# Chengyuann/AutoStyle-TTS

Hardware: AMD Instinct MI355X
Metric: synthesized audio sec/wall-sec (RTF^-1) + style-kNN QPS, IEMOCAP test batch (higher is better)
Workload: dtype f16; 1 GPU; BASELINE configs[1]: batch=8 utterances/GPU, kNN Q=8 x N=1000 x D=6144 k=3, synthesis Tt=32 Tp=150 Ts=250 (fixed-length decode, EOS ignored) -> 430 mel frames -> 110080 samples @ 22050 Hz; CosyVoice-300M shapes, random-init weights; parallelism=dp1 (model + bank replicated, utterances sharded, all-gather of style ids only)

## Files before the change

### autostyle-tts_amd/astts/_lib_session.py

```python
from __future__ import annotations

import functools
import os

from . import _lib

HEADER_PATH = os.path.normpath(os.path.join(os.path.dirname(os.path.abspath(__file__)), "..", "..", "include", "session",
                                            "astts_lm_session.h"))


@functools.lru_cache(maxsize=None)
def signatures() -> dict:
    if not os.path.exists(HEADER_PATH):
        raise _lib.AsttsLibraryMissing(f"{HEADER_PATH} not found: the ctypes signatures of the session calls are derived from this header")
    with open(HEADER_PATH) as f:
        return _lib.parse_prototypes(f.read())


@functools.lru_cache(maxsize=None)
def load():
    lib = _lib.load()
    for name, (res, args) in signatures().items():
        fn = getattr(lib, name)
        fn.restype = res
        fn.argtypes = args
    return lib
```

### autostyle-tts_amd/astts/synth/flow.py

```python
from __future__ import annotations

import ctypes
import math
from typing import List, NamedTuple, Optional

import torch

from .. import _lib, ops
from ..ops import PackedWeight
from .config import SynthConfig
from .encoder import SD, RelPosEncoder, _dev, fold_layernorm


class _Resnet1D:
    def __init__(self, sd: SD, p: str, device, groups: int):
        self.groups = groups
        self.c1 = PackedWeight.from_conv1d(sd[p + ".block1.block.0.weight"], sd[p + ".block1.block.0.bias"], device)
        self.g1 = (_dev(sd[p + ".block1.block.1.weight"], device), _dev(sd[p + ".block1.block.1.bias"], device))
        self.mlp = PackedWeight(sd[p + ".mlp.1.weight"], sd[p + ".mlp.1.bias"], device)
        self.c2 = PackedWeight.from_conv1d(sd[p + ".block2.block.0.weight"], sd[p + ".block2.block.0.bias"], device)
        self.g2 = (_dev(sd[p + ".block2.block.1.weight"], device), _dev(sd[p + ".block2.block.1.bias"], device))
        self.res = PackedWeight.from_conv1d(sd[p + ".res_conv.weight"], sd[p + ".res_conv.bias"], device)
        self.fused = all(w.cin == w.cin_pad for w in (self.c1, self.c2, self.res)) and \
            ops.resnet_conv_supported(self.c1.cin, self.c1.n, groups, self.c1.taps) and \
            ops.resnet_conv_supported(self.c2.cin, self.c2.n, groups, self.c2.taps) and \
            ops.resnet_conv_supported(self.res.cin, self.res.n, groups, self.res.taps)
        self.c1_frag, self.c2_frag, self.res_frag = ((ops.conv_pack_frag(self.c1), ops.conv_pack_frag(self.c2), ops.conv_pack_frag(self.res))
                                                     if self.fused else (None, None, None))

    def forward(self, x: torch.Tensor, lens: torch.Tensor, temb_mish: torch.Tensor, tproj: Optional[torch.Tensor] = None) -> torch.Tensor:
        if tproj is None:
            tproj = ops.linear(temb_mish, self.mlp)
        if self.fused:
            x = x.contiguous()
            h1, s1 = ops.resnet_conv(x, self.c1, self.c1_frag, lens=lens, want_stats=True)
            h2, s2 = ops.resnet_conv(h1, self.c2, self.c2_frag, lens=lens, in_gn=(s1, *self.g1), in_add=tproj.contiguous(), want_stats=True)
            return ops.resnet_conv(x, self.res, self.res_frag, lens=lens, res_gn=(h2, s2, *self.g2))
        h = ops.conv1d(x, self.c1, pad=1)
        h = ops.groupnorm(h, *self.g1, self.groups, 1e-5, lens=lens, mish=True, add_bc=tproj, out_dtype=torch.float16)
        h = ops.conv1d(h, self.c2, pad=1)
        h = ops.groupnorm(h, *self.g2, self.groups, 1e-5, lens=lens, mish=True)
        return ops.conv1d(x, self.res, residual=h)


class _TfmBlock:
    def __init__(self, sd: SD, p: str, heads: int, device):
        self.heads = heads
        wqkv = torch.cat([sd[p + ".attn1.to_q.weight"], sd[p + ".attn1.to_k.weight"], sd[p + ".attn1.to_v.weight"]], 0).float().cpu()
        wqkv, bqkv = fold_layernorm(wqkv, torch.zeros(wqkv.shape[0]), sd[p + ".norm1.weight"].float().cpu(), sd[p + ".norm1.bias"].float().cpu())
        c = int(wqkv.shape[1])
        self.n1 = (torch.ones(c, dtype=torch.float32, device=device), torch.zeros(c, dtype=torch.float32, device=device))
        self.wqkv = PackedWeight(wqkv, bqkv, device)
        self.wqkv_frag = ops.tfm_pack_frag(self.wqkv) if c == 256 and wqkv.shape[0] % 32 == 0 else None
        self.wo = PackedWeight(sd[p + ".attn1.to_out.0.weight"], sd[p + ".attn1.to_out.0.bias"], device)
        w1, b1 = fold_layernorm(sd[p + ".ff.net.0.proj.weight"].float().cpu(), sd[p + ".ff.net.0.proj.bias"].float().cpu(),
                                sd[p + ".norm3.weight"].float().cpu(), sd[p + ".norm3.bias"].float().cpu())
        self.n3 = self.n1
        self.w1 = PackedWeight(w1, b1, device)
        self.w2 = PackedWeight(sd[p + ".ff.net.2.weight"], sd[p + ".ff.net.2.bias"], device)
        self.ffn_fused = ops.tfm_ffn_fused_supported(c, int(w1.shape[0]))
        self.w1_frag = ops.tfm_pack_frag(self.w1) if self.ffn_fused else None
        self.w2_frag = ops.tfm_pack_frag(self.w2) if self.ffn_fused else None
        self.wo_frag = ops.tfm_pack_frag(self.wo) if self.ffn_fused and self.wo.cin in (256, 512) else None

    def forward(self, x: torch.Tensor, lens: torch.Tensor) -> torch.Tensor:
        hd = self.heads * 64
        f16 = torch.float16
        if self.wqkv_frag is not None and ops.tfm_attn_fused_supported(x.shape[-1], self.heads, x.shape[1]):
            a = ops.tfm_attn_fused(x, self.wqkv, self.wqkv_frag, self.heads, lens=lens, eps=1e-5)
        else:
            n = ops.layernorm(x, *self.n1, 1e-5, out_dtype=f16)
            qkv = ops.linear(n, self.wqkv, out_dtype=f16)
            a = ops.attn_mha(qkv[..., :hd], qkv[..., hd:2 * hd], qkv[..., 2 * hd:], self.heads, lens=lens, out_dtype=f16)
        if self.wo_frag is not None:
            return ops.tfm_ffn_fused(x, self.w1, self.w1_frag, self.w2, self.w2_frag, eps=1e-5, attn=a.contiguous(), wo=self.wo, wo_frag=self.wo_frag)
        x = ops.linear(a, self.wo, residual=x)
        if self.ffn_fused:
            return ops.tfm_ffn_fused(x, self.w1, self.w1_frag, self.w2, self.w2_frag, eps=1e-5)
        n = ops.layernorm(x, *self.n3, 1e-5, out_dtype=f16)
        f = ops.linear(n, self.w1, act="gelu", out_dtype=f16)
        return ops.linear(f, self.w2, residual=x)


class _Block(NamedTuple):
    res: _Resnet1D
    tfms: List[_TfmBlock]
    resample: Optional[PackedWeight] = None
    last: bool = False


class FlowDecoder:

    def __init__(self, sd: SD, cfg: SynthConfig, device):
        self.cfg, self.device = cfg, device
        self.use_engine = True
        self.tok_emb = _dev(sd["input_embedding.weight"], device)
        self.spk_aff = PackedWeight(sd["spk_embed_affine_layer.weight"], sd["spk_embed_affine_layer.bias"], device)
        self.enc = RelPosEncoder(sd, "encoder", cfg.flow_heads, cfg.flow_layers, "swish", ("norm_mha", "norm_ff"), False,
                                 False, cfg.ln_eps, cfg.max_positions, device)
        self.enc_proj = PackedWeight(sd["encoder_proj.weight"], sd["encoder_proj.bias"], device)
        self.lr = []
        for j in range(4):
            self.lr.append((PackedWeight.from_conv1d(sd[f"length_regulator.model.{3 * j}.weight"],
                                                     sd[f"length_regulator.model.{3 * j}.bias"], device),
                            _dev(sd[f"length_regulator.model.{3 * j + 1}.weight"], device),
                            _dev(sd[f"length_regulator.model.{3 * j + 1}.bias"], device)))
        self.lr_out = PackedWeight.from_conv1d(sd["length_regulator.model.12.weight"], sd["length_regulator.model.12.bias"], device)
        e = "decoder.estimator"
        self.t1 = PackedWeight(sd[e + ".time_mlp.linear_1.weight"], sd[e + ".time_mlp.linear_1.bias"], device)
        self.t2 = PackedWeight(sd[e + ".time_mlp.linear_2.weight"], sd[e + ".time_mlp.linear_2.bias"], device)
        ch = cfg.est_channels
        g = cfg.est_groups
        self.down, self.mid, self.up = [], [], []
        for i in range(len(ch)):
            p = f"{e}.down_blocks.{i}"
            last = i == len(ch) - 1
            wname = p + ".2" + ("" if last else ".conv")
            self.down.append(_Block(_Resnet1D(sd, p + ".0", device, g),
                                    [_TfmBlock(sd, f"{p}.1.{j}", cfg.est_heads, device) for j in range(cfg.est_tfm_per_block)],
                                    PackedWeight.from_conv1d(sd[wname + ".weight"], sd[wname + ".bias"], device), last))
        for i in range(cfg.est_mid_blocks):
            p = f"{e}.mid_blocks.{i}"
            self.mid.append(_Block(_Resnet1D(sd, p + ".0", device, g),
                                   [_TfmBlock(sd, f"{p}.1.{j}", cfg.est_heads, device) for j in range(cfg.est_tfm_per_block)]))
        for i in range(len(ch)):
            p = f"{e}.up_blocks.{i}"
            last = i == len(ch) - 1
            if last:
                w = PackedWeight.from_conv1d(sd[p + ".2.weight"], sd[p + ".2.bias"], device)
            else:
                w = PackedWeight.from_conv_transpose1d(sd[p + ".2.conv.weight"], sd[p + ".2.conv.bias"], 2, device)
            self.up.append(_Block(_Resnet1D(sd, p + ".0", device, g),
                                  [_TfmBlock(sd, f"{p}.1.{j}", cfg.est_heads, device) for j in range(cfg.est_tfm_per_block)], w, last))
        self.fin_c = PackedWeight.from_conv1d(sd[e + ".final_block.block.0.weight"], sd[e + ".final_block.block.0.bias"], device)
        self.fin_g = (_dev(sd[e + ".final_block.block.1.weight"], device), _dev(sd[e + ".final_block.block.1.bias"], device))
        self.fin_p = PackedWeight.from_conv1d(sd[e + ".final_proj.weight"], sd[e + ".final_proj.bias"], device)

    def mu(self, tokens: torch.Tensor, token_lens: torch.Tensor, mel_total: int, mel_lens: Optional[torch.Tensor] = None) -> torch.Tensor:
        x = ops.embedding(self.tok_emb, tokens.clamp(min=0))
        x = ops.elementwise(ops.EL_MUL_ROWMASK, x, lens=token_lens)
        h = ops.linear(self.enc.forward(x, token_lens), self.enc_proj)
        h = ops.interp_linear(h, mel_total, in_lens=None if mel_lens is None else token_lens, out_lens=mel_lens)
        for w, ga, be in self.lr:
            h = ops.conv1d(h, w, pad=1)
            h = ops.groupnorm(h, ga, be, 1, 1e-5, lens=mel_lens, mish=True)
        h = ops.conv1d(h, self.lr_out)
        return h if mel_lens is None else ops.elementwise(ops.EL_MUL_ROWMASK, h, lens=mel_lens)

    def time_path(self, t: torch.Tensor) -> List[torch.Tensor]:
        temb = ops.time_embedding(t, self.cfg.est_in)
        temb = ops.linear(ops.linear(temb, self.t1, act="silu"), self.t2)
        temb_m = ops.elementwise(ops.EL_MISH, temb)
        return [ops.linear(temb_m, blk.res.mlp) for grp in (self.down, self.mid, self.up) for blk in grp]

    def estimator(self, x, mu, spk, cond, t, lens, full: bool = False, tprojs: Optional[List[torch.Tensor]] = None) -> torch.Tensor:
        cfg = self.cfg
        b, T, _ = x.shape
        if full:
            _mask = lambda h, L: h
        else:
            _mask = lambda h, L: ops.elementwise(ops.EL_MUL_ROWMASK, h, lens=L)
        if tprojs is None:
            tprojs = self.time_path(t)
        tp = iter(tprojs)
        temb_m = None
        h = torch.cat([x, mu, spk[:, None, :].expand(b, T, -1), cond], dim=-1)
        hiddens, lens_stack = [], [lens]
        for res, tfms, wds, last in self.down:
            L = lens_stack[-1]
            h = _mask(h, L)
            h = res.forward(h, L, temb_m, next(tp))
            for tb in tfms:
                h = tb.forward(h, L)
            hiddens.append(h)
            hm = _mask(h, L)
            if last:
                h = ops.conv1d(hm, wds, pad=1)
                lens_stack.append(L)
            else:
                h = ops.conv1d(hm, wds, stride=2, pad=1)
                lens_stack.append(torch.div(L + 1, 2, rounding_mode="floor").to(torch.int32))
        L = lens_stack[-1]
        h = _mask(h, L)
        for blk in self.mid:
            h = blk.res.forward(h, L, temb_m, next(tp))
            for tb in blk.tfms:
                h = tb.forward(h, L)
            h = _mask(h, L)
        lens_stack.pop()
        for res, tfms, wus, last in self.up:
            L = lens_stack.pop()
            skip = hiddens.pop()
            h = torch.cat([h[:, :skip.shape[1]], skip], dim=-1)
            h = _mask(h, L)
            h = res.forward(h, L, temb_m, next(tp))
            for tb in tfms:
                h = tb.forward(h, L)
            hm = _mask(h, L)
            if last:
                h = ops.conv1d(hm, wus, pad=1)
            else:
                h = ops.conv_transpose1d(hm, wus, padding=1)
        h = _mask(h[:, :T].contiguous(), lens)
        h = ops.conv1d(h, self.fin_c, pad=1)
        h = ops.groupnorm(h, *self.fin_g, cfg.est_groups, 1e-5, lens=lens, mish=True)
        out = ops.conv1d(h, self.fin_p)
        return _mask(out, lens)

    def _engine(self):
        if getattr(self, "_eng", None) is None:
            cfg = self.cfg
            keep = []

            def W(pw):
                return ops.Weight(pw.data.data_ptr(), None if pw.bias is None else pw.bias.data_ptr(), pw.n, pw.cin, pw.cin_pad, pw.taps)

            def R(r):
                fp = [None if f is None else f.data_ptr() for f in (r.c1_frag, r.c2_frag, r.res_frag)]
                return ops.FlowResnet(W(r.c1), W(r.mlp), W(r.c2), W(r.res), r.g1[0].data_ptr(), r.g1[1].data_ptr(),
                                      r.g2[0].data_ptr(), r.g2[1].data_ptr(), *fp)

            def TF(tfms):
                arr = (ops.FlowTfm * len(tfms))()
                for i, t in enumerate(tfms):
                    arr[i] = ops.FlowTfm(t.n1[0].data_ptr(), t.n1[1].data_ptr(), t.n3[0].data_ptr(), t.n3[1].data_ptr(),
                                         W(t.wqkv), W(t.wo), W(t.w1), W(t.w2), None if t.wqkv_frag is None else t.wqkv_frag.data_ptr(),
                                         None if t.w1_frag is None else t.w1_frag.data_ptr(), None if t.w2_frag is None else t.w2_frag.data_ptr(),
                                         None if t.wo_frag is None else t.wo_frag.data_ptr())
                keep.append(arr)
                return arr

            def blocks(items, kinds):
                arr = (ops.FlowBlock * max(len(items), 1))()
                for i, (blk, kind) in enumerate(zip(items, kinds)):
                    rs = W(blk.resample) if kind != ops.FLOW_RESAMPLE_NONE else ops.Weight()
                    arr[i] = ops.FlowBlock(R(blk.res), TF(blk.tfms), len(blk.tfms), rs, kind)
                keep.append(arr)
                return arr

            down = blocks(self.down, [ops.FLOW_RESAMPLE_CONV if blk.last else ops.FLOW_RESAMPLE_DOWN for blk in self.down])
            mid = blocks(self.mid, [ops.FLOW_RESAMPLE_NONE] * len(self.mid))
            up = blocks(self.up, [ops.FLOW_RESAMPLE_CONV if blk.last else ops.FLOW_RESAMPLE_UP for blk in self.up])
            c = ops.FlowConfig(cfg.mel, cfg.est_channels[0], cfg.est_heads, cfg.est_groups, cfg.est_in, cfg.est_time_dim,
                               len(self.down), len(self.mid), len(self.up), W(self.t1), W(self.t2), W(self.fin_c), W(self.fin_p),
                               self.fin_g[0].data_ptr(), self.fin_g[1].data_ptr())
            h = ctypes.c_void_p()
            _lib.check(_lib.load().astts_flow_create(ctypes.byref(c), down, mid, up, ctypes.byref(h)))
            self._eng, self._eng_keep = h, keep
        return self._eng

    def _schedule(self):
        n = self.cfg.cfm_steps
        ts = 1.0 - torch.cos(torch.linspace(0, 1, n + 1) * 0.5 * math.pi)
        return [float(ts[s]) for s in range(n)], [float(ts[s + 1] - ts[s]) for s in range(n)]

    def solve(self, x: torch.Tensor, mu: torch.Tensor, spk_e: torch.Tensor, cond: torch.Tensor,
              lens: Optional[torch.Tensor] = None) -> torch.Tensor:
        lib = _lib.load()
        eng = self._engine()
        b, t, _ = x.shape
        assert x.is_contiguous() and mu.is_contiguous() and cond.is_contiguous() and spk_e.is_contiguous()
        assert x.dtype == mu.dtype == cond.dtype == spk_e.dtype == torch.float32
        tv, dv = self._schedule()
        n = len(tv)
        need = int(lib.astts_flow_workspace_bytes(eng, b, t))
        ws = torch.empty(need, dtype=torch.uint8, device=x.device)
        _lib.check(lib.astts_flow_solve(eng, x.data_ptr(), mu.data_ptr(), spk_e.data_ptr(), cond.data_ptr(),
                                        None if lens is None else lens.data_ptr(), b, t, n, (ctypes.c_float * n)(*tv),
                                        (ctypes.c_float * n)(*dv), self.cfg.cfg_rate, ws.data_ptr(), need,
                                        _lib.stream_ptr()))
        return x

    def solve_ops(self, x, mu, spk_e, cond, lens: Optional[torch.Tensor] = None) -> torch.Tensor:
        b, t, _ = x.shape
        full = lens is None
        if full:
            lens = torch.full((b,), t, dtype=torch.int32, device=x.device)
        lens2 = torch.cat([lens, lens])
        mu2 = torch.cat([mu, torch.zeros_like(mu)], 0)
        spk2 = torch.cat([spk_e, torch.zeros_like(spk_e)], 0)
        cond2 = torch.cat([cond, torch.zeros_like(cond)], 0)
        tv, dv = self._schedule()
        b2 = 2 * b
        t_all = torch.tensor(tv, dtype=torch.float32, device=x.device).repeat_interleave(b2)
        tp_all = self.time_path(t_all)
        for s in range(len(tv)):
            t2 = t_all[s * b2:(s + 1) * b2]
            d = self.estimator(torch.cat([x, x], 0), mu2, spk2, cond2, t2, lens2, full=full,
                               tprojs=[tp[s * b2:(s + 1) * b2] for tp in tp_all])
            x = ops.elementwise(ops.EL_CFG_EULER, x, z=d, s=dv[s], s2=self.cfg.cfg_rate)
        return x

    def decode(self, tokens, token_lens, prompt_mel, spk, z, mel_total: int) -> torch.Tensor:
        cfg = self.cfg
        b = tokens.shape[0]
        mu = self.mu(tokens, token_lens, mel_total)
        spk_e = ops.linear(torch.nn.functional.normalize(spk, dim=1), self.spk_aff)
        tmp = prompt_mel.shape[1]
        cond = torch.zeros((b, mel_total, cfg.mel), dtype=torch.float32, device=self.device)
        cond[:, :tmp] = prompt_mel
        x = (self.solve if self.use_engine else self.solve_ops)(z.clone(), mu, spk_e, cond)
        return x[:, tmp:].contiguous()

    def decode_ragged(self, tokens: List[torch.Tensor], prompt_mels: List[torch.Tensor], spk: torch.Tensor,
                      zs: List[torch.Tensor]) -> List[torch.Tensor]:
        cfg, dev = self.cfg, self.device
        b = len(tokens)
        tl = [int(t.numel()) for t in tokens]
        tmp = [int(m.shape[0]) for m in prompt_mels]
        mt = [int(z.shape[0]) for z in zs]
        tmax, mmax = max(tl), max(mt)
        tok = torch.zeros((b, tmax), dtype=torch.int32, device=dev)
        cond = torch.zeros((b, mmax, cfg.mel), dtype=torch.float32, device=dev)
        x = torch.zeros((b, mmax, cfg.mel), dtype=torch.float32, device=dev)
        for i in range(b):
            tok[i, :tl[i]] = tokens[i].to(dev).view(-1)
            cond[i, :tmp[i]] = prompt_mels[i].to(dev)
            x[i, :mt[i]] = zs[i].to(dev)
        tok_lens = torch.tensor(tl, dtype=torch.int32, device=dev)
        mel_lens = torch.tensor(mt, dtype=torch.int32, device=dev)
        mu = self.mu(tok, tok_lens, mmax, mel_lens)
        spk_e = ops.linear(torch.nn.functional.normalize(spk.to(dev), dim=1), self.spk_aff)
        x = (self.solve if self.use_engine else self.solve_ops)(x, mu, spk_e, cond, mel_lens)
        return [x[i, tmp[i]:mt[i]].contiguous() for i in range(b)]
```

### autostyle-tts_amd/astts/synth/pipeline.py

```python
from __future__ import annotations

import os
import threading
import time
from collections import deque
from concurrent.futures import Future, ThreadPoolExecutor
from typing import List, NamedTuple, Optional, Tuple

import torch

from .. import _lib, ops
from .decode import Prefill, record_streams
from .lm import AcousticLM

Slot = Optional[Tuple[int, int]]


def plan_streams(class_sizes: List[int], depth: int) -> Tuple[Slot, List[Slot], Slot]:
    n = len(class_sizes)
    if n >= depth + 2:
        return (0, 0), [(c, 0) for c in range(1, depth + 1)], (depth + 1, 0)
    front = (0, 1) if class_sizes[0] > 1 else None
    lm_classes = list(range(1, n)) if n > 1 else [0]
    lm = []
    for i in range(depth):
        c = lm_classes[i % len(lm_classes)]
        j = i // len(lm_classes) + (0 if n > 1 else 2)
        lm.append((c, j) if j < class_sizes[c] else None)
    return (0, 0), lm, front


class LmArgs(NamedTuple):
    text: torch.Tensor
    text_lens: torch.Tensor
    lm_spk: torch.Tensor
    lm_prompt_tokens: torch.Tensor
    n_tokens: int
    uniforms: torch.Tensor

    @property
    def rows(self) -> int:
        return int(self.text.shape[0])

    @classmethod
    def concat(cls, parts: List["LmArgs"]) -> "LmArgs":
        a = parts
        return cls(torch.cat([x.text for x in a], 0), torch.cat([x.text_lens for x in a], 0), torch.cat([x.lm_spk for x in a], 0),
                   torch.cat([x.lm_prompt_tokens for x in a], 0), a[0].n_tokens, torch.cat([x.uniforms for x in a], 1))


def _lib_check_spin(us: int, stream) -> None:
    _lib.check(_lib.load().astts_stream_spin(int(us), int(stream.cuda_stream)))


class _JoinChain:

    ROWS_MAX = 16

    def __init__(self, lm, device, stream, index: int, quantum: int, ahead: int, max_window: int):
        self.lm, self.device, self.stream, self.index = lm, device, stream, index
        self.quantum, self.ahead, self.max_window = quantum, ahead, max_window
        self.session = None
        self._cv = threading.Condition()
        self._waiting = deque()
        self._occupied = 0
        self._half = 0
        self._stop = False
        self._dead = None
        self._thread = None
        self.gate = threading.Event()
        self.gate.set()
        self.joins = 0

    def occupied(self) -> int:
        with self._cv:
            return self._occupied

    def reserve(self, window: int) -> bool:
        with self._cv:
            if self._dead is not None:
                raise RuntimeError(f"decode chain {self.index} stopped: {self._dead!r}") from self._dead
            if self._occupied >= 2 or window > self.max_window:
                return False
            if window > self._half:
                if self._occupied:
                    return False
                self._half = min((window + 127) // 128 * 128, self.max_window)
            self._occupied += 1
            return True

    def submit(self, state: Prefill, lm_args: LmArgs) -> Future:
        cur = torch.cuda.current_stream(self.device)
        record_streams(lm_args, self.stream)
        record_streams(state.tensors(), self.stream)
        ready = torch.cuda.Event()
        ready.record(cur)
        fut = Future()
        with self._cv:
            if self._dead is not None:
                self._occupied -= 1
                raise RuntimeError(f"decode chain {self.index} stopped: {self._dead!r}") from self._dead
            self._waiting.append((state, lm_args.uniforms, ready, fut))
            if self._thread is None:
                self._thread = threading.Thread(target=self._run, name=f"astts-join-chain-{self.index}", daemon=True)
                self._thread.start()
            self._cv.notify()
        return fut

    def close(self) -> None:
        with self._cv:
            self._stop = True
            self._cv.notify()
        self.gate.set()
        if self._thread is not None:
            self._thread.join()
            self._thread = None
        if self.session is not None:
            self.session.close()
            self.session = None

    def _admit_waiting(self, futs) -> None:
        while True:
            with self._cv:
                if not self._waiting:
                    return
                state, u, ready, fut = self._waiting[0]
                half = self._half
            idle = self.session is None or not self.session.active()
            if idle and (self.session is None or self.session.max_window < half):
                if self.session is not None:
                    self.session.close()
                    self.session = None
                self.session = self.lm.session(self.ROWS_MAX, 2 * half, self.stream)
            if not self.session.can_admit(state.b, state.s0, state.n_steps):
                if not idle:
                    return
                with self._cv:
                    self._waiting.popleft()
                    self._occupied -= 1
                fut.set_exception(RuntimeError(f"decode chain {self.index}: a batch of {state.b} rows with a window of "
                                               f"{state.s0 + state.n_steps - 1} keys does not fit a session of {self.ROWS_MAX} rows "
                                               f"and {self.session.max_window} keys"))
                continue
            self.joins += 0 if idle else 1
            self.stream.wait_event(ready)
            futs[id(self.session.admit(state, u, ignore_eos=True))] = fut
            with self._cv:
                self._waiting.popleft()

    def _run(self):
        ahead = deque()
        futs = {}
        try:
            with torch.cuda.device(self.device), torch.cuda.stream(self.stream):
                while True:
                    self.gate.wait()
                    with self._cv:
                        while not self._stop and not self._waiting and not (self.session is not None and self.session.active()):
                            self._cv.wait()
                        if self._stop:
                            return
                    self._admit_waiting(futs)
                    if not self.session.active():
                        continue
                    done = self.session.step(min(self.quantum, min(self.session.steps_left())))
                    mark = torch.cuda.Event()
                    mark.record(self.stream)
                    for job in done:
                        with self._cv:
                            self._occupied -= 1
                        futs.pop(id(job)).set_result(([job.toks], mark))
                    ahead.append(mark)
                    if len(ahead) > self.ahead:
                        ahead.popleft().synchronize()
        except BaseException as e:
            with self._cv:
                self._dead = e
                pending = [w[3] for w in self._waiting]
                self._waiting.clear()
                self._occupied = 0
            for f in list(futs.values()) + pending:
                if not f.done():
                    f.set_exception(e)


class PipelinedSynth:

    JOIN_QUANTUM = 16
    JOIN_AHEAD = 2

    def __init__(self, engine, lm_depth: int = 2, lm_priority: int = -1, render_priority: int = 0, streams=None,
                 cobatch: int = 1, render_depth: int = 1, pipe_classes=None, front_prefill: Optional[bool] = None,
                 stagger_ms: Optional[float] = None, wide_lm: bool = False, join: bool = False):
        self.eng = engine
        self.depth = max(1, int(lm_depth))
        self.render_depth = rd = max(1, int(render_depth))
        dev = engine.device
        with torch.cuda.device(dev):
            self.front_stream = None
            extra_render = []
            if streams is not None:
                self.s_lm, self.s_render = list(streams[:self.depth]), streams[self.depth]
                extra_render = list(streams[self.depth + 1:self.depth + rd])
            elif lm_priority != render_priority:
                self.s_lm = [torch.cuda.Stream(device=dev, priority=lm_priority) for _ in range(self.depth)]
                self.s_render = torch.cuda.Stream(device=dev, priority=render_priority)
            elif rd > 1:
                st = ops.concurrent_streams(self.depth + 1 + rd, priority=lm_priority, device=dev)
                self.s_render, extra_render, self.front_stream, self.s_lm = st[0], st[1:rd], st[rd], st[rd + 1:]
            else:
                classes = pipe_classes if pipe_classes is not None else ops.stream_pipe_classes(priority=lm_priority, device=dev)
                render, lm, front = plan_streams([len(c) for c in classes], self.depth)
                self.s_render = classes[render[0]][render[1]]
                self.s_lm = [torch.cuda.Stream(device=dev, priority=lm_priority) if s is None else classes[s[0]][s[1]] for s in lm]
                self.front_stream = None if front is None else classes[front[0]][front[1]]
            if self.front_stream is None:
                self.front_stream = torch.cuda.Stream(device=dev)
            while len(extra_render) < rd - 1:
                extra_render.append(torch.cuda.Stream(device=dev, priority=render_priority))
            self.s_renders = [self.s_render] + list(extra_render)
            self._r = 0
        self._pool = ThreadPoolExecutor(max_workers=self.depth)
        self._fifo = deque()
        self._pending = []
        self.cobatch = max(1, int(cobatch))
        self.wide_lm = bool(wide_lm)
        self.lm_rows_max = AcousticLM.WIDE_ROWS if self.wide_lm else 32
        self.front_prefill = (os.environ.get("ASTTS_PIPE_FRONT_PREFILL", "1") != "0") if front_prefill is None else bool(front_prefill)
        self.stagger_ms = float(os.environ.get("ASTTS_PIPE_STAGGER_MS", "0")) if stagger_ms is None else float(stagger_ms)
        self._staggered = set()
        self._i = 0
        self.join = bool(join) and self.cobatch == 1 and not self.wide_lm
        lm_ = engine.lm
        self._chains = [_JoinChain(lm_, dev, self.s_lm[c], c, self.JOIN_QUANTUM, self.JOIN_AHEAD, lm_.body.center)
                        for c in range(self.depth)] if self.join else []

    def close(self) -> None:
        for ch in self._chains:
            ch.close()
        self._chains = []
        self._pool.shutdown(wait=True)

    @classmethod
    def autotune(cls, engine, sample_args, depths=(3, 2), trials: int = 3, steps: int = 4, verbose: bool = False,
                 front=None, dist=None, wide_lm: bool = False):
        best, best_dt = None, float("inf")
        per_cfg = []
        with torch.cuda.device(engine.device):
            classes = ops.stream_pipe_classes(device=engine.device, verbose=verbose)
        tried = []
        for cfg_ in depths:
            cfg_ = cfg_ if isinstance(cfg_, tuple) else (cfg_, 1)
            for join in (False, True):
                if join and (cfg_[1] != 1 or wide_lm):
                    continue
                tried.append(tuple(cfg_) + ("join",) if join else cfg_)
        for cfg_ in tried:
            join = cfg_[-1] == "join"
            depth, cob, rdep = (tuple(cfg_[:-1] if join else cfg_) + (1,))[:3]
            for _ in range(trials):
                lm_prio = int(os.environ.get("ASTTS_PIPE_LM_PRIORITY", "0"))
                pipe = cls(engine, lm_depth=depth, lm_priority=lm_prio, render_priority=0, cobatch=cob, render_depth=rdep,
                           pipe_classes=classes if rdep == 1 and lm_prio == 0 else None, wide_lm=wide_lm, join=join)
                with torch.cuda.stream(pipe.front_stream):
                    for _ in range((depth + 1) * cob):
                        if front is not None:
                            front()
                        pipe.submit(*sample_args)
                    pipe.drain()
                    torch.cuda.synchronize(engine.device)
                    t0 = time.perf_counter()
                    for _ in range(steps):
                        if front is not None:
                            front()
                        pipe.submit(*sample_args)
                    pipe.drain()
                    torch.cuda.synchronize(engine.device)
                dt = (time.perf_counter() - t0) / steps
                if verbose:
                    print(f"PipelinedSynth.autotune: depth {depth} cobatch {cob} render streams {rdep} join {join}: {dt * 1e3:.1f} ms/batch", flush=True)
                if dt < best_dt:
                    best, best_dt = pipe, dt
                if not per_cfg or per_cfg[-1][2] != cfg_:
                    per_cfg.append([pipe, dt, cfg_])
                elif dt < per_cfg[-1][1]:
                    if per_cfg[-1][0] is not best:
                        per_cfg[-1][0].close()
                    per_cfg[-1][0], per_cfg[-1][1] = pipe, dt
                else:
                    pipe.close()
        if dist is not None and len(per_cfg) > 1:
            t = torch.tensor([c[1] for c in per_cfg], dtype=torch.float64, device=engine.device)
            dist.all_reduce(t, op=dist.ReduceOp.MAX)
            k = int(torch.argmin(t).item())
            best, best_dt = per_cfg[k][0], per_cfg[k][1]
            best.tuned_agreed_over_ranks = True
        for c in per_cfg:
            if c[0] is not best:
                c[0].close()
        best.tuned_ms_per_batch = best_dt * 1e3
        best.tuned_table_ms = {str(c[2]): round(c[1] * 1e3, 2) for c in per_cfg}
        return best

    def _launch_group(self):
        group, self._pending = self._pending, []
        chain = self._i % self.depth
        stream = self.s_lm[chain]
        self._i += 1
        cur = torch.cuda.current_stream(self.eng.device)
        if self.stagger_ms > 0 and chain > 0 and chain not in self._staggered:
            self._staggered.add(chain)
            us = int(self.stagger_ms * 1000.0 * chain)
            while us > 0:
                _lib_check_spin(min(us, 100000), stream)
                us -= 100000
        lm_args = group[0]["lm"] if len(group) == 1 else LmArgs.concat([g["lm"] for g in group])
        record_streams(lm_args, stream)
        sizes = [g["lm"].rows for g in group]
        state = None
        if self.front_prefill and sum(sizes) <= self.lm_rows_max:
            state = self.eng.tts_prefill(*lm_args[:5])
            record_streams(state.tensors(), stream)
        stream.wait_stream(cur)

        def lm_stage():
            with torch.cuda.device(self.eng.device), torch.cuda.stream(stream):
                toks = self.eng.tts_tokens(*lm_args, wide=self.wide_lm) if state is None else self.eng.tts_decode(state, lm_args.uniforms)
                parts = list(torch.split(toks, sizes, 0)) if len(sizes) > 1 else [toks]
                ev = torch.cuda.Event()
                ev.record(stream)
            return parts, ev

        fut = self._pool.submit(lm_stage)
        for k, g in enumerate(group):
            g["fut"], g["k"] = fut, k

    def _render(self, item):
        parts, ev = item["fut"].result()
        toks = parts[item["k"]]
        cur = torch.cuda.current_stream(self.eng.device)
        sr = self.s_renders[self._r % self.render_depth]
        self._r += 1
        with torch.cuda.stream(sr):
            sr.wait_event(ev)
            toks.record_stream(sr)
            record_streams(item["render"], sr)
            mel, wav = self.eng.tts_render(toks, *item["render"])
        record_streams((toks, mel, wav), cur)
        return toks, mel, wav

    def submit(self, text, text_lens, lm_spk, lm_prompt_tokens, n_tokens, uniforms, flow_prompt_tokens, flow_prompt_mel,
               flow_spk, z, phase0, noise):
        cur = torch.cuda.current_stream(self.eng.device)
        for sr in self.s_renders:
            sr.wait_stream(cur)
        item = {"lm": LmArgs(text, text_lens, lm_spk, lm_prompt_tokens, n_tokens, uniforms),
                "render": (flow_prompt_tokens, flow_prompt_mel, flow_spk, z, phase0, noise), "fut": None, "k": 0}
        if self.join and self._join_submit(item):
            return self._render(self._fifo.popleft()) if len(self._fifo) > 2 * self.depth else None
        if self._pending and not self._compatible(self._pending[0]["lm"], item["lm"]):
            self._launch_group()
        self._pending.append(item)
        self._fifo.append(item)
        if len(self._pending) >= self.cobatch:
            self._launch_group()
        if len(self._fifo) > self.depth * self.cobatch and self._fifo[0]["fut"] is not None:
            return self._render(self._fifo.popleft())
        return None

    def _join_submit(self, item) -> bool:
        lm, lm_args = self.eng.lm, item["lm"]
        if lm_args.rows > _JoinChain.ROWS_MAX // 2:
            return False
        pre = lm.prefix(lm_args.text, lm_args.text_lens, lm_args.lm_spk, lm_args.lm_prompt_tokens)
        window = int(pre.shape[0]) + int(lm_args.n_tokens) - 1
        if window > lm.body.center:
            return False
        state = lm.prefill(pre, lm_args.n_tokens)
        order = lambda: sorted(self._chains, key=lambda ch: (ch.occupied() != 1, ch.index))
        chain = next((ch for ch in order() if ch.reserve(window)), None)
        for older in list(self._fifo):
            if chain is not None:
                break
            if older["fut"] is not None:
                try:
                    older["fut"].result()
                except Exception:
                    pass
                chain = next((ch for ch in order() if ch.reserve(window)), None)
        if chain is None:
            raise RuntimeError("PipelinedSynth: no decode chain can take the batch although none holds one")
        self._fifo.append(item)
        item["fut"] = chain.submit(state, lm_args)
        return True

    def _compatible(self, a: LmArgs, b: LmArgs) -> bool:
        return (a.n_tokens == b.n_tokens and a.text.shape[1] == b.text.shape[1]
                and a.lm_prompt_tokens.shape[1] == b.lm_prompt_tokens.shape[1] and a.uniforms.shape[0] == b.uniforms.shape[0]
                and a.rows + b.rows <= self.lm_rows_max)

    def drain(self):
        if self._pending:
            self._launch_group()
        self._staggered = set()
        self._i = 0
        out = []
        while self._fifo:
            out.append(self._render(self._fifo.popleft()))
        cur = torch.cuda.current_stream(self.eng.device)
        for st in self.s_lm:
            cur.wait_stream(st)
        for sr in self.s_renders:
            cur.wait_stream(sr)
        return out
```

### autostyle-tts_amd/csrc/flow_engine.hip

```cpp
#include "common.h"

#include <vector>

struct astts_flow {
    astts_flow_config_t cfg;
    struct Block {
        astts_flow_resnet_t res;
        std::vector<astts_flow_tfm_t> tfm;
        astts_weight_t resample;
        int kind;
    };
    std::vector<Block> down, mid, up;
};

namespace astts {

__global__ __launch_bounds__(256) void flow_pack_input(const float* __restrict__ x, const float* __restrict__ mu,
                                                      const float* __restrict__ spk, const float* __restrict__ cond,
                                                      const int* __restrict__ lens2, float* __restrict__ out, int b, int t,
                                                      int mel) {
    const int c4 = 4 * mel;
    const int64_t total = (int64_t)2 * b * t * c4;
    for (int64_t i = (int64_t)blockIdx.x * blockDim.x + threadIdx.x; i < total; i += (int64_t)gridDim.x * blockDim.x) {
        const int c = (int)(i % c4);
        const int64_t row = i / c4;
        const int bb = (int)(row / t), tt = (int)(row % t);
        const int src_b = bb < b ? bb : bb - b;
        const int part = c / mel, cc = c % mel;
        float v = 0.0f;
        if (tt < lens2[bb]) {
            const int64_t o = ((int64_t)src_b * t + tt) * mel + cc;
            if (part == 0) v = x[o];
            else if (bb < b) v = part == 1 ? mu[o] : (part == 2 ? spk[(int64_t)src_b * mel + cc] : cond[o]);
        }
        out[i] = v;
    }
}

__global__ __launch_bounds__(256) void flow_concat_skip(const float* __restrict__ a, int64_t a_bs, const float* __restrict__ skip,
                                                       const int* __restrict__ lens, float* __restrict__ out, int b2, int t, int c) {
    const int c4 = c / 4;
    const int64_t total = (int64_t)b2 * t * 2 * c4;
    for (int64_t i = (int64_t)blockIdx.x * blockDim.x + threadIdx.x; i < total; i += (int64_t)gridDim.x * blockDim.x) {
        const int cc = (int)(i % (2 * c4));
        const int64_t row = i / (2 * c4);
        const int bb = (int)(row / t), tt = (int)(row % t);
        float4 v = make_float4(0.f, 0.f, 0.f, 0.f);
        if (tt < lens[bb]) {
            if (cc < c4) v = reinterpret_cast<const float4*>(a + (int64_t)bb * a_bs + (int64_t)tt * c)[cc];
            else v = reinterpret_cast<const float4*>(skip + row * c)[cc - c4];
        }
        reinterpret_cast<float4*>(out)[i] = v;
    }
}

__global__ void flow_fill_lens(const int* __restrict__ lens, int* __restrict__ lens_full, int* __restrict__ lens_half, int b, int t) {
    const int i = blockIdx.x * blockDim.x + threadIdx.x;
    if (i < 2 * b) {
        const int l = lens ? lens[i < b ? i : i - b] : t;
        lens_full[i] = l;
        lens_half[i] = (l + 1) / 2;
    }
}

__global__ void flow_fill_time(float* __restrict__ tv, float value, int n) {
    const int i = blockIdx.x * blockDim.x + threadIdx.x;
    if (i < n) tv[i] = value;
}

static inline int grid_for(int64_t total) {
    int64_t g = (total + 255) / 256;
    return (int)(g > 8192 ? 8192 : g);
}

}

using namespace astts;

#define RUN(expr)                          \
    do {                                   \
        const int rc_ = (expr);            \
        if (rc_ != ASTTS_OK) return rc_;   \
    } while (0)

namespace {

constexpr int FLOW_MAX_STEPS = 32;

struct Buffers {
    float *xin, *r1, *r2, *r3, *pool[6], *temb0, *temb1, *temb2, *tproj, *tv, *d, *up;
    _Float16 *r1h, *n16, *qkv16, *a16, *f16;
    int *lens_full, *lens_half;
    void* gn_ws;
    size_t gn_ws_bytes;
    float *rstat1, *rstat2;
};

size_t carve(const astts_flow* h, int b, int t, char* base, Buffers* B) {
    const astts_flow_config_t& c = h->cfg;
    const size_t b2 = 2 * (size_t)b, rows = b2 * t, C = c.channels, hd = (size_t)c.heads * 64;
    size_t o = 0;
    auto take = [&](size_t bytes) {
        void* p = base ? base + o : nullptr;
        o = align_up(o + bytes, 256);
        return p;
    };
    const size_t in_ch = 4 * (size_t)c.mel > 2 * C ? 4 * (size_t)c.mel : 2 * C;
    Buffers tmp;
    Buffers& X = B ? *B : tmp;
    X.xin = (float*)take(sizeof(float) * rows * in_ch);
    X.r1 = (float*)take(sizeof(float) * rows * C);
    X.r2 = (float*)take(sizeof(float) * rows * C);
    X.r3 = (float*)take(sizeof(float) * rows * C);
    for (int i = 0; i < 6; ++i) X.pool[i] = (float*)take(sizeof(float) * rows * C);
    X.up = (float*)take(sizeof(float) * b2 * ((size_t)t + 4) * 2 * C);
    X.r1h = (_Float16*)take(sizeof(_Float16) * rows * C);
    X.n16 = (_Float16*)take(sizeof(_Float16) * rows * C);
    X.qkv16 = (_Float16*)take(sizeof(_Float16) * rows * 3 * hd);
    X.a16 = (_Float16*)take(sizeof(_Float16) * rows * hd);
    X.f16 = (_Float16*)take(sizeof(_Float16) * rows * 4 * C);
    const size_t n_res = h->down.size() + h->mid.size() + h->up.size();
    X.temb0 = (float*)take(sizeof(float) * FLOW_MAX_STEPS * b2 * c.time_in);
    X.temb1 = (float*)take(sizeof(float) * FLOW_MAX_STEPS * b2 * c.time_dim);
    X.temb2 = (float*)take(sizeof(float) * FLOW_MAX_STEPS * b2 * c.time_dim);
    X.tproj = (float*)take(sizeof(float) * n_res * FLOW_MAX_STEPS * b2 * C);
    X.tv = (float*)take(sizeof(float) * FLOW_MAX_STEPS * b2);
    X.d = (float*)take(sizeof(float) * rows * c.mel);
    X.lens_full = (int*)take(sizeof(int) * b2);
    X.lens_half = (int*)take(sizeof(int) * b2);
    X.gn_ws_bytes = astts_op_groupnorm_workspace_bytes((int)b2, t, c.groups);
    X.gn_ws = take(X.gn_ws_bytes > 16 ? X.gn_ws_bytes : 16);
    X.rstat1 = (float*)take(sizeof(float) * astts_op_resnet_conv_stats_floats((int32_t)b2, t));
    X.rstat2 = (float*)take(sizeof(float) * astts_op_resnet_conv_stats_floats((int32_t)b2, t));
    return o;
}

struct Ctx {
    const astts_flow* h;
    Buffers B;
    int b2, T;
    bool full;
    astts_stream_t st;

    int gemm(const void* x, int x16, const astts_weight_t& w, const float* residual, void* out, int out16, int64_t m,
             int t_in, int t_out, int stride, int pad, int act) const {
        return astts_op_gemm(x, x16, w.w, w.bias, residual, nullptr, out, out16, m, w.n, w.cin, w.cin_pad, w.taps, w.cin, w.n,
                             residual ? w.n : 0, t_in, t_out, stride, 1, pad, act, 1.0f, 0.1f, nullptr, st);
    }
    int linear(const void* x, int x16, const astts_weight_t& w, const float* residual, void* out, int out16, int64_t m, int act) const {
        return gemm(x, x16, w, residual, out, out16, m, (int)m, (int)m, 1, 0, act);
    }
    int mask(float* x, const int* lens, int t, int c) const {
        if (full) return ASTTS_OK;
        return astts_op_elementwise(ASTTS_EL_MUL_ROWMASK, x, nullptr, nullptr, lens, x, (int64_t)b2 * t * c, t, c, 0.0f, 0.0f, st);
    }

    int resnet(const astts_flow_resnet_t& r, const float* tproj, const float* x, const int* lens, int t, float* out,
               const void* next_w = nullptr, uint32_t next_bytes = 0) const {
        const int C = h->cfg.channels, G = h->cfg.groups;
        const int64_t rows = (int64_t)b2 * t;
        if (r.c1_frag && r.c2_frag && r.res_frag && astts_op_resnet_conv_supported(r.c1.cin, r.c1.n, G, r.c1.taps) &&
            astts_op_resnet_conv_supported(r.c2.cin, r.c2.n, G, r.c2.taps) && astts_op_resnet_conv_supported(r.res.cin, r.res.n, G, r.res.taps)) {
            auto wbytes = [](const astts_weight_t& w) { return (uint32_t)((size_t)w.n * w.taps * w.cin_pad * 2); };
            RUN(astts_op_resnet_conv(x, r.c1_frag, r.c1.bias, B.r1, nullptr, nullptr, nullptr, nullptr, nullptr, nullptr, nullptr, nullptr,
                                     B.rstat1, lens, b2, t, r.c1.cin, r.c1.taps, 1e-5f, r.c2_frag, wbytes(r.c2), st));
            RUN(astts_op_resnet_conv(B.r1, r.c2_frag, r.c2.bias, B.r2, B.rstat1, r.g1_w, r.g1_b, tproj, nullptr, nullptr, nullptr, nullptr,
                                     B.rstat2, lens, b2, t, r.c2.cin, r.c2.taps, 1e-5f, r.res_frag, wbytes(r.res), st));
            return astts_op_resnet_conv(x, r.res_frag, r.res.bias, out, nullptr, nullptr, nullptr, nullptr, B.r2, B.rstat2, r.g2_w, r.g2_b,
                                        nullptr, lens, b2, t, r.res.cin, r.res.taps, 1e-5f, next_w, next_bytes, st);
        }
        RUN(gemm(x, 0, r.c1, nullptr, B.r1, 0, rows, t, t, 1, 1, ASTTS_ACT_NONE));
        RUN(astts_op_groupnorm(B.r1, lens, r.g1_w, r.g1_b, tproj, B.r1h, 1, b2, t, C, G, 1e-5f, 1, B.gn_ws, B.gn_ws_bytes, st));
        RUN(gemm(B.r1h, 1, r.c2, nullptr, B.r2, 0, rows, t, t, 1, 1, ASTTS_ACT_NONE));
        RUN(astts_op_groupnorm(B.r2, lens, r.g2_w, r.g2_b, nullptr, B.r3, 0, b2, t, C, G, 1e-5f, 1, B.gn_ws, B.gn_ws_bytes, st));
        return gemm(x, 0, r.res, B.r3, out, 0, rows, t, t, 1, 0, ASTTS_ACT_NONE);
    }

    int tfm(const astts_flow_tfm_t& w, float* p, float* q, const int* lens, int t, const void* next_w = nullptr, uint32_t next_bytes = 0) const {
        const int C = h->cfg.channels, heads = h->cfg.heads, hd = heads * 64;
        const int64_t rows = (int64_t)b2 * t;
        static const int64_t unfused_min = exp_env_int("ASTTS_FLOW_UNFUSED_ATTN_MIN_ROWS", 0);
        const bool fused_attn = w.qkv_frag && astts_op_tfm_attn_fused_supported(C, heads, t) && !(unfused_min > 0 && rows >= unfused_min);
        if (fused_attn) {
            const void* pf[3] = {w.wo_frag, w.w1_frag, w.w2_frag};
            const uint32_t pfb[3] = {(uint32_t)((size_t)C * hd * 2), (uint32_t)((size_t)w.w1.n * C * 2), (uint32_t)((size_t)C * w.w1.n * 2)};
            RUN(astts_op_tfm_attn_fused(p, w.qkv_frag, w.qkv.bias, lens, B.a16, b2, heads, t, C, 1e-5f, 0.125f, pf, pfb,
                                        (w.wo_frag && w.w1_frag && w.w2_frag) ? 3 : 0, st));
        } else {
            RUN(astts_op_layernorm(p, w.n1_w, w.n1_b, B.n16, 1, rows, C, C, C, 1e-5f, 0.0f, st));
            RUN(linear(B.n16, 1, w.qkv, nullptr, B.qkv16, 1, rows, ASTTS_ACT_NONE));
            RUN(astts_op_attn_mha(B.qkv16, B.qkv16 + hd, B.qkv16 + 2 * hd, 1, lens, B.a16, 1, b2, heads, t, 3 * hd, 3 * hd, hd,
                                  0.125f, st));
        }
        const bool ffn = w.w1_frag && w.w2_frag && astts_op_tfm_ffn_fused_supported(C, w.w1.n);
        if (ffn && w.wo_frag && (hd == 256 || hd == 512))
            return astts_op_tfm_ffn_fused(p, w.w1_frag, w.w1.bias, w.w2_frag, w.w2.bias, p, rows, C, w.w1.n, 1e-5f, B.a16, w.wo_frag,
                                          w.wo.bias, hd, next_w, next_bytes, st);
        RUN(linear(B.a16, 1, w.wo, p, q, 0, rows, ASTTS_ACT_NONE));
        if (ffn)
            return astts_op_tfm_ffn_fused(q, w.w1_frag, w.w1.bias, w.w2_frag, w.w2.bias, p, rows, C, w.w1.n, 1e-5f, nullptr, nullptr, nullptr, 0, nullptr, 0,
                                          st);
        RUN(astts_op_layernorm(q, w.n3_w, w.n3_b, B.n16, 1, rows, C, C, C, 1e-5f, 0.0f, st));
        RUN(linear(B.n16, 1, w.w1, nullptr, B.f16, 1, rows, ASTTS_ACT_GELU));
        return linear(B.f16, 1, w.w2, q, p, 0, rows, ASTTS_ACT_NONE);
    }
};

}

extern "C" {

int astts_flow_create(const astts_flow_config_t* cfg, const astts_flow_block_t* down, const astts_flow_block_t* mid,
                      const astts_flow_block_t* up, astts_flow_t** out) {
    ASTTS_REQUIRE(cfg && down && mid && up && out, ASTTS_ERR_INVALID, "astts_flow_create: null argument");
    ASTTS_REQUIRE(cfg->mel >= 1 && cfg->channels >= 64 && cfg->channels % 64 == 0 && cfg->heads >= 1 && cfg->groups >= 1 &&
                      cfg->channels % cfg->groups == 0, ASTTS_ERR_INVALID, "astts_flow_create: bad sizes");
    ASTTS_REQUIRE(cfg->n_down >= 1 && cfg->n_down <= 4 && cfg->n_up == cfg->n_down && cfg->n_mid >= 0, ASTTS_ERR_INVALID,
                  "astts_flow_create: n_down=%d n_mid=%d n_up=%d", cfg->n_down, cfg->n_mid, cfg->n_up);
    int n_half = 0;
    for (int i = 0; i < cfg->n_down; ++i) n_half += down[i].resample_kind == ASTTS_FLOW_RESAMPLE_DOWN;
    ASTTS_REQUIRE(n_half <= 1, ASTTS_ERR_UNSUPPORTED, "astts_flow_create: more than one stride-2 level is not implemented");
    ASTTS_REQUIRE(down[cfg->n_down - 1].resample_kind == ASTTS_FLOW_RESAMPLE_CONV && up[cfg->n_up - 1].resample_kind == ASTTS_FLOW_RESAMPLE_CONV,
                  ASTTS_ERR_UNSUPPORTED, "astts_flow_create: the last down / up block must end in the k=3 convolution");
    astts_flow* h = new astts_flow();
    h->cfg = *cfg;
    auto copy = [](const astts_flow_block_t* src, int n, std::vector<astts_flow::Block>& dst) {
        for (int i = 0; i < n; ++i) {
            astts_flow::Block blk;
            blk.res = src[i].res;
            blk.tfm.assign(src[i].tfm, src[i].tfm + src[i].n_tfm);
            blk.resample = src[i].resample;
            blk.kind = src[i].resample_kind;
            dst.push_back(blk);
        }
    };
    copy(down, cfg->n_down, h->down);
    copy(mid, cfg->n_mid, h->mid);
    copy(up, cfg->n_up, h->up);
    *out = h;
    return ASTTS_OK;
}

int astts_flow_destroy(astts_flow_t* h) {
    delete h;
    return ASTTS_OK;
}

size_t astts_flow_workspace_bytes(const astts_flow_t* h, int32_t b, int32_t t) {
    if (!h || b < 1 || t < 1) return 0;
    return carve(h, b, t, nullptr, nullptr);
}

int astts_flow_solve(astts_flow_t* h, float* x, const float* mu, const float* spk, const float* cond, const int32_t* lens,
                     int32_t b, int32_t t, int32_t n_steps, const float* t_host, const float* dt_host, float cfg_rate,
                     void* workspace, size_t workspace_bytes, astts_stream_t stream) {
    ASTTS_REQUIRE(h && x && mu && spk && cond && t_host && dt_host && workspace, ASTTS_ERR_INVALID, "astts_flow_solve: null argument");
    ASTTS_REQUIRE(b >= 1 && t >= 2 && n_steps >= 1, ASTTS_ERR_INVALID, "astts_flow_solve: b=%d t=%d n_steps=%d", b, t, n_steps);
    ASTTS_REQUIRE(workspace_bytes >= astts_flow_workspace_bytes(h, b, t) && ((uintptr_t)workspace & 255) == 0,
                  ASTTS_ERR_WORKSPACE, "astts_flow_solve: workspace too small or misaligned");
    const astts_flow_config_t& c = h->cfg;
    hipStream_t st = (hipStream_t)stream;
    Ctx k;
    k.h = h;
    k.b2 = 2 * b;
    k.T = t;
    k.full = lens == nullptr;
    k.st = stream;
    carve(h, b, t, (char*)workspace, &k.B);
    const Buffers& B = k.B;
    const int b2 = k.b2, C = c.channels, mel = c.mel;
    const int t_half = (t - 1) / 2 + 1;

    hipLaunchKernelGGL(flow_fill_lens, dim3((b2 + 63) / 64), dim3(64), 0, st, lens, B.lens_full, B.lens_half, b, t);
    ASTTS_CHECK_LAUNCH();

    for (int s = 0; s < n_steps; ++s) {
      const int s0 = s - s % FLOW_MAX_STEPS, sl = s - s0;
      const int64_t trows = (int64_t)(n_steps - s0 < FLOW_MAX_STEPS ? n_steps - s0 : FLOW_MAX_STEPS) * b2;
      if (sl == 0) {
        for (int j = 0; j < (int)(trows / b2); ++j) {
            hipLaunchKernelGGL(flow_fill_time, dim3((b2 + 63) / 64), dim3(64), 0, st, B.tv + (size_t)j * b2, t_host[s0 + j], b2);
            ASTTS_CHECK_LAUNCH();
        }
        RUN(astts_op_time_embedding(B.tv, B.temb0, (int)trows, c.time_in, 1000.0f, st));
        RUN(k.linear(B.temb0, 0, c.t1, nullptr, B.temb1, 0, trows, ASTTS_ACT_SILU));
        RUN(k.linear(B.temb1, 0, c.t2, nullptr, B.temb2, 0, trows, ASTTS_ACT_NONE));
        RUN(astts_op_elementwise(ASTTS_EL_MISH, B.temb2, nullptr, nullptr, nullptr, B.temb2, trows * c.time_dim, 1, c.time_dim, 0.0f, 0.0f, st));
        size_t rj = 0;
        for (const std::vector<astts_flow::Block>* grp : {&h->down, &h->mid, &h->up})
            for (const astts_flow::Block& blk : *grp)
                RUN(k.linear(B.temb2, 0, blk.res.mlp, nullptr, B.tproj + (rj++) * (size_t)trows * C, 0, trows, ASTTS_ACT_NONE));
      }
      {
        size_t ri = 0;
        auto tproj_of = [&]() { return B.tproj + ((ri++) * (size_t)trows + (size_t)sl * b2) * C; };
        hipLaunchKernelGGL(flow_pack_input, dim3(grid_for((int64_t)b2 * t * 4 * mel)), dim3(256), 0, st, x, mu, spk, cond,
                           B.lens_full, B.xin, b, t, mel);
        ASTTS_CHECK_LAUNCH();

        float* pool[6];
        for (int i = 0; i < 6; ++i) pool[i] = B.pool[i];
        int n_free = 6;
        auto grab = [&]() { return pool[--n_free]; };
        float* cur = grab();
        float* other = grab();
        float* skips[4];
        int skip_t[4];
        const int* skip_lens[4];
        int n_skips = 0;
        const float* block_in = B.xin;
        int tt = t;
        const int* L = B.lens_full;

        const uint32_t qkv_bytes = 3u * (uint32_t)c.heads * 64u * (uint32_t)C * 2u;
        for (size_t i = 0; i < h->down.size(); ++i) {
            const astts_flow::Block& blk = h->down[i];
            RUN(k.resnet(blk.res, tproj_of(), block_in, L, tt, other, blk.tfm.empty() ? nullptr : blk.tfm[0].qkv_frag, qkv_bytes));
            { float* sw = cur; cur = other; other = sw; }
            for (size_t ti = 0; ti < blk.tfm.size(); ++ti) {
                const bool more = ti + 1 < blk.tfm.size();
                RUN(k.tfm(blk.tfm[ti], cur, other, L, tt, more ? blk.tfm[ti + 1].qkv_frag : nullptr,
                          more ? (uint32_t)(3u * (uint32_t)c.heads * 64u * (uint32_t)C * 2u) : 0u));
            }
            RUN(k.mask(cur, L, tt, C));
            skips[n_skips] = cur;
            skip_t[n_skips] = tt;
            skip_lens[n_skips] = L;
            ++n_skips;
            float* nxt = other;
            other = grab();
            if (blk.kind == ASTTS_FLOW_RESAMPLE_DOWN) {
                RUN(k.gemm(cur, 0, blk.resample, nullptr, nxt, 0, (int64_t)b2 * t_half, tt, t_half, 2, 1, ASTTS_ACT_NONE));
                tt = t_half;
                L = B.lens_half;
            } else {
                RUN(k.gemm(cur, 0, blk.resample, nullptr, nxt, 0, (int64_t)b2 * tt, tt, tt, 1, 1, ASTTS_ACT_NONE));
            }
            cur = nxt;
            RUN(k.mask(cur, L, tt, C));
            block_in = cur;
        }
        for (size_t mi = 0; mi < h->mid.size(); ++mi) {
            const astts_flow::Block& blk = h->mid[mi];
            RUN(k.resnet(blk.res, tproj_of(), cur, L, tt, other, blk.tfm.empty() ? nullptr : blk.tfm[0].qkv_frag, qkv_bytes));
            float* sw = cur; cur = other; other = sw;
            for (size_t ti = 0; ti < blk.tfm.size(); ++ti) {
                const bool more = ti + 1 < blk.tfm.size();
                const astts_flow_resnet_t* nr = (!more && mi + 1 < h->mid.size()) ? &h->mid[mi + 1].res : nullptr;
                const astts_weight_t* nc = nr ? &nr->c1 : nullptr;
                const void* nw = !nr ? nullptr
                                 : (nr->c1_frag && nr->c2_frag && nr->res_frag && astts_op_resnet_conv_supported(nc->cin, nc->n, c.groups, nc->taps) &&
                                    astts_op_resnet_conv_supported(nr->c2.cin, nr->c2.n, c.groups, nr->c2.taps) &&
                                    astts_op_resnet_conv_supported(nr->res.cin, nr->res.n, c.groups, nr->res.taps)) ? nr->c1_frag : nc->w;
                RUN(k.tfm(blk.tfm[ti], cur, other, L, tt, more ? blk.tfm[ti + 1].qkv_frag : nw,
                          more ? (uint32_t)(3u * (uint32_t)c.heads * 64u * (uint32_t)C * 2u)
                               : (nc ? (uint32_t)((size_t)nc->n * nc->taps * nc->cin_pad * 2) : 0u)));
            }
            RUN(k.mask(cur, L, tt, C));
        }
        const float* up_src = cur;
        int64_t up_bs = (int64_t)tt * C;
        for (size_t i = 0; i < h->up.size(); ++i) {
            const astts_flow::Block& blk = h->up[i];
            --n_skips;
            tt = skip_t[n_skips];
            L = skip_lens[n_skips];
            hipLaunchKernelGGL(flow_concat_skip, dim3(grid_for((int64_t)b2 * tt * 2 * (C / 4))), dim3(256), 0, st, up_src, up_bs,
                               skips[n_skips], L, B.xin, b2, tt, C);
            ASTTS_CHECK_LAUNCH();
            RUN(k.resnet(blk.res, tproj_of(), B.xin, L, tt, cur, blk.tfm.empty() ? nullptr : blk.tfm[0].qkv_frag, qkv_bytes));
            for (size_t ti = 0; ti < blk.tfm.size(); ++ti) {
                const bool more = ti + 1 < blk.tfm.size();
                RUN(k.tfm(blk.tfm[ti], cur, other, L, tt, more ? blk.tfm[ti + 1].qkv_frag : nullptr,
                          more ? (uint32_t)(3u * (uint32_t)c.heads * 64u * (uint32_t)C * 2u) : 0u));
            }
            RUN(k.mask(cur, L, tt, C));
            if (blk.kind == ASTTS_FLOW_RESAMPLE_UP) {
                RUN(k.gemm(cur, 0, blk.resample, nullptr, B.up, 0, (int64_t)b2 * (tt + 1), tt, tt + 1, 1, 1, ASTTS_ACT_NONE));
                up_src = B.up + C;
                up_bs = (int64_t)(tt + 1) * 2 * C;
            } else {
                RUN(k.gemm(cur, 0, blk.resample, nullptr, other, 0, (int64_t)b2 * tt, tt, tt, 1, 1, ASTTS_ACT_NONE));
                float* sw = cur; cur = other; other = sw;
                up_src = cur;
                up_bs = (int64_t)tt * C;
            }
        }
        float* fin = const_cast<float*>(up_src);
        RUN(k.mask(fin, B.lens_full, t, C));
        RUN(k.gemm(fin, 0, c.fin_c, nullptr, B.r1, 0, (int64_t)b2 * t, t, t, 1, 1, ASTTS_ACT_NONE));
        RUN(astts_op_groupnorm(B.r1, B.lens_full, c.fin_g_w, c.fin_g_b, nullptr, B.r3, 0, b2, t, C, c.groups, 1e-5f, 1, B.gn_ws,
                               B.gn_ws_bytes, st));
        RUN(k.gemm(B.r3, 0, c.fin_p, nullptr, B.d, 0, (int64_t)b2 * t, t, t, 1, 0, ASTTS_ACT_NONE));
        RUN(k.mask(B.d, B.lens_full, t, mel));
        RUN(astts_op_elementwise(ASTTS_EL_CFG_EULER, x, B.d, nullptr, nullptr, x, (int64_t)b * t * mel, t, mel, dt_host[s], cfg_rate, st));
      }
    }
    return ASTTS_OK;
}

}
```

Before: 521.8 audio-s/wall-s.

## Add continuous-batching flow session that joins render jobs across estimator passes

Adds a native flow-matching session holding up to four in-flight render jobs. Each estimator pass runs over all active jobs' rows together, and a new job can be admitted mid-solve. A background render thread feeds finished LM outputs into this session instead of running a separate full ODE solve per batch. The goal is larger, better-filled estimator GEMMs and less serialization between LM and render stages. The cost is extra threading, a per-pass join/assemble kernel and host-side scheduling overhead. It is only active in autotune candidates that pick render_join.

After: 537.4 audio-s/wall-s (median of 6 runs). 1.03x the previous value.

```diff
diff --git a/autostyle-tts_amd/astts/_lib_session.py b/autostyle-tts_amd/astts/_lib_session.py
--- a/autostyle-tts_amd/astts/_lib_session.py
+++ b/autostyle-tts_amd/astts/_lib_session.py
@@ -5,16 +5,20 @@
 
 from . import _lib
 
-HEADER_PATH = os.path.normpath(os.path.join(os.path.dirname(os.path.abspath(__file__)), "..", "..", "include", "session",
-                                            "astts_lm_session.h"))
+_DIR = os.path.normpath(os.path.join(os.path.dirname(os.path.abspath(__file__)), "..", "..", "include", "session"))
+HEADER_PATH = os.path.join(_DIR, "astts_lm_session.h")
+FLOW_HEADER_PATH = os.path.join(_DIR, "astts_flow_session.h")
 
 
 @functools.lru_cache(maxsize=None)
 def signatures() -> dict:
-    if not os.path.exists(HEADER_PATH):
-        raise _lib.AsttsLibraryMissing(f"{HEADER_PATH} not found: the ctypes signatures of the session calls are derived from this header")
-    with open(HEADER_PATH) as f:
-        return _lib.parse_prototypes(f.read())
+    sigs = {}
+    for path in (HEADER_PATH, FLOW_HEADER_PATH):
+        if not os.path.exists(path):
+            raise _lib.AsttsLibraryMissing(f"{path} not found: the ctypes signatures of the session calls are derived from this header")
+        with open(path) as f:
+            sigs.update(_lib.parse_prototypes(f.read()))
+    return sigs
 
 
 @functools.lru_cache(maxsize=None)
diff --git a/autostyle-tts_amd/astts/synth/flow.py b/autostyle-tts_amd/astts/synth/flow.py
--- a/autostyle-tts_amd/astts/synth/flow.py
+++ b/autostyle-tts_amd/astts/synth/flow.py
@@ -302,6 +302,18 @@
         x = (self.solve if self.use_engine else self.solve_ops)(z.clone(), mu, spk_e, cond)
         return x[:, tmp:].contiguous()
 
+    def session(self, t: int, slots: int = 4, rows_max: int = 32, stream=None) -> "FlowSession":
+        return FlowSession(self, t, slots, rows_max, stream)
+
+    def prepare(self, tokens, token_lens, prompt_mel, spk, z, mel_total: int):
+        b = tokens.shape[0]
+        mu = self.mu(tokens, token_lens, mel_total)
+        spk_e = ops.linear(torch.nn.functional.normalize(spk, dim=1), self.spk_aff)
+        tmp = prompt_mel.shape[1]
+        cond = torch.zeros((b, mel_total, self.cfg.mel), dtype=torch.float32, device=self.device)
+        cond[:, :tmp] = prompt_mel
+        return z.clone(), mu, spk_e, cond, tmp
+
     def decode_ragged(self, tokens: List[torch.Tensor], prompt_mels: List[torch.Tensor], spk: torch.Tensor,
                       zs: List[torch.Tensor]) -> List[torch.Tensor]:
         cfg, dev = self.cfg, self.device
@@ -323,3 +335,85 @@
         spk_e = ops.linear(torch.nn.functional.normalize(spk.to(dev), dim=1), self.spk_aff)
         x = (self.solve if self.use_engine else self.solve_ops)(x, mu, spk_e, cond, mel_lens)
         return [x[i, tmp[i]:mt[i]].contiguous() for i in range(b)]
+
+
+class FlowJob:
+
+    def __init__(self, x, mu, spk_e, cond, lens, n_steps: int):
+        self.x, self.mu, self.spk_e, self.cond, self.lens = x, mu, spk_e, cond, lens
+        self.n_steps, self.next, self.slot = int(n_steps), 0, -1
+
+
+class FlowSession:
+
+    def __init__(self, flow: FlowDecoder, t: int, slots: int = 4, rows_max: int = 32, stream=None):
+        from .. import _lib_session
+        self.flow, self.t, self.slots, self.rows_max = flow, int(t), int(slots), int(rows_max)
+        self.stream = stream if stream is not None else torch.cuda.current_stream(flow.device)
+        self._lib = _lib_session.load()
+        self._tv, self._dv = flow._schedule()
+        eng = flow._engine()
+        need = int(self._lib.astts_flow_session_bytes(eng, self.t, self.slots, self.rows_max, len(self._tv)))
+        if need == 0:
+            raise ValueError(f"FlowSession: t={t} slots={slots} rows_max={rows_max} steps={len(self._tv)}")
+        with torch.cuda.stream(self.stream):
+            self._ws = torch.empty(need, dtype=torch.uint8, device=flow.device)
+        h = ctypes.c_void_p()
+        _lib.check(self._lib.astts_flow_session_create(eng, self.t, self.slots, self.rows_max, len(self._tv), self._ws.data_ptr(), need,
+                                                       _lib.stream_ptr(self.stream), ctypes.byref(h)))
+        self._h = h
+        self._ctx: List[Optional[FlowJob]] = [None] * 4
+
+    def close(self) -> None:
+        if self._h is not None:
+            h, self._h = self._h, None
+            _lib.check(self._lib.astts_flow_session_destroy(h))
+
+    def active(self) -> int:
+        return sum(c is not None for c in self._ctx)
+
+    def steps_left(self) -> List[int]:
+        return [c.n_steps - c.next for c in self._ctx if c is not None]
+
+    def can_admit(self, b: int, t: int) -> bool:
+        return int(self._lib.astts_flow_session_can_admit(self._h, int(b), int(t), len(self._tv))) >= 0
+
+    def state(self) -> List[int]:
+        out = (ctypes.c_int32 * 8)()
+        _lib.check(self._lib.astts_flow_session_state(self._h, out))
+        return list(out)
+
+    def admit(self, x: torch.Tensor, mu: torch.Tensor, spk_e: torch.Tensor, cond: torch.Tensor,
+              lens: Optional[torch.Tensor] = None) -> FlowJob:
+        b, t, _ = x.shape
+        assert x.is_contiguous() and mu.is_contiguous() and cond.is_contiguous() and spk_e.is_contiguous()
+        assert x.dtype == mu.dtype == cond.dtype == spk_e.dtype == torch.float32
+        n = len(self._tv)
+        job = FlowJob(x, mu, spk_e, cond, lens, n)
+        slot = ctypes.c_int32(-1)
+        with torch.cuda.stream(self.stream):
+            _lib.check(self._lib.astts_flow_session_admit(self._h, x.data_ptr(), mu.data_ptr(), spk_e.data_ptr(), cond.data_ptr(),
+                                                          None if lens is None else lens.data_ptr(), b, t, n, (ctypes.c_float * n)(*self._tv),
+                                                          (ctypes.c_float * n)(*self._dv), self.flow.cfg.cfg_rate, ctypes.byref(slot)))
+        job.slot = int(slot.value)
+        self._ctx[job.slot] = job
+        return job
+
+    def step(self, k: int = 1) -> List[FlowJob]:
+        mask = ctypes.c_uint32(0)
+        k = int(k)
+        with torch.cuda.stream(self.stream):
+            _lib.check(self._lib.astts_flow_session_step(self._h, k, ctypes.byref(mask)))
+        done = []
+        for slot, c in enumerate(self._ctx):
+            if c is None:
+                continue
+            c.next = min(c.n_steps, c.next + k)
+            if mask.value >> slot & 1:
+                done.append(c)
+                self._ctx[slot] = None
+        return done
+
+    def run(self) -> None:
+        while self.active():
+            self.step(max(self.steps_left()))
diff --git a/autostyle-tts_amd/astts/synth/pipeline.py b/autostyle-tts_amd/astts/synth/pipeline.py
--- a/autostyle-tts_amd/astts/synth/pipeline.py
+++ b/autostyle-tts_amd/astts/synth/pipeline.py
@@ -184,14 +184,145 @@
                     f.set_exception(e)
 
 
+class _JoinRender:
+
+    SLOTS, ROWS_MAX, AHEAD = 4, 32, 2
+
+    def __init__(self, engine, stream):
+        self.eng, self.device, self.stream = engine, engine.device, stream
+        self.session = None
+        self._cv = threading.Condition()
+        self._waiting = []
+        self._stop = False
+        self._dead = None
+        self._thread = None
+        self.passes = self.carried = 0
+        self.gate = threading.Event()
+        self.gate.set()
+
+    def submit(self, item, ready) -> None:
+        item["rfut"], item["ready"] = Future(), ready
+        with self._cv:
+            if self._dead is not None:
+                raise RuntimeError(f"render worker stopped: {self._dead!r}") from self._dead
+            self._waiting.append(item)
+            if self._thread is None:
+                self._thread = threading.Thread(target=self._run, name="astts-join-render", daemon=True)
+                self._thread.start()
+        item["fut"].add_done_callback(self._wake)
+
+    def _wake(self, _fut=None) -> None:
+        with self._cv:
+            self._cv.notify()
+
+    def stats(self):
+        s = self.session.state() if self.session is not None else [0] * 8
+        return self.passes + s[2], self.carried + s[3]
+
+    def close(self) -> None:
+        with self._cv:
+            self._stop = True
+            self._cv.notify()
+        self.gate.set()
+        if self._thread is not None:
+            self._thread.join()
+            self._thread = None
+        self._drop_session()
+
+    def _drop_session(self) -> None:
+        if self.session is not None:
+            self.passes, self.carried = self.stats()
+            self.session.close()
+            self.session = None
+
+    def _take_ready(self):
+        busy = self.session is not None and self.session.active() > 0
+        with self._cv:
+            for i, item in enumerate(self._waiting):
+                fut = item["fut"]
+                if fut.done() and (not busy or fut.exception() is not None or fut.result()[1].query()):
+                    return self._waiting.pop(i)
+        return None
+
+    def _begin(self, item, jobs) -> None:
+        eng, sr = self.eng, self.stream
+        try:
+            parts, ev = item["fut"].result()
+        except Exception as e:
+            item["rfut"].set_exception(e)
+            return
+        toks = parts[item["k"]]
+        sr.wait_event(ev)
+        sr.wait_event(item["ready"])
+        toks.record_stream(sr)
+        record_streams(item["render"], sr)
+        ptok, pmel, spk, z, phase0, noise = item["render"]
+        b = int(toks.shape[0])
+        mel_total = int(pmel.shape[1]) + eng.cfg.mel_frames_for_tokens(toks.shape[1])
+        idle = self.session is None or not self.session.active()
+        if idle and b <= self.ROWS_MAX and (self.session is None or self.session.t != mel_total):
+            self._drop_session()
+            self.session = eng.flow.session(mel_total, self.SLOTS, self.ROWS_MAX, sr)
+        if not eng.flow.use_engine or self.session is None or not self.session.can_admit(b, mel_total):
+            mel, wav = eng.tts_render(toks, *item["render"])
+            item["rfut"].set_result((toks, mel, wav))
+            return
+        all_tok = torch.cat([ptok.to(torch.int32), toks], dim=1)
+        tok_lens = torch.full((b,), all_tok.shape[1], dtype=torch.int32, device=self.device)
+        x, mu, spk_e, cond, tmp = eng.flow.prepare(all_tok, tok_lens, pmel, spk, z, mel_total)
+        jobs[id(self.session.admit(x, mu, spk_e, cond))] = (item, toks, tmp)
+
+    def _run(self):
+        ahead = deque()
+        jobs = {}
+        item = None
+        try:
+            with torch.cuda.device(self.device), torch.cuda.stream(self.stream):
+                while True:
+                    self.gate.wait()
+                    with self._cv:
+                        while not self._stop and not (self.session is not None and self.session.active()) and \
+                                not any(w["fut"].done() for w in self._waiting):
+                            self._cv.wait()
+                        if self._stop:
+                            return
+                    while True:
+                        item = self._take_ready()
+                        if item is None:
+                            break
+                        self._begin(item, jobs)
+                        item = None
+                    if self.session is None or not self.session.active():
+                        continue
+                    for job in self.session.step(1):
+                        it, toks, tmp = jobs.pop(id(job))
+                        mel = job.x[:, tmp:].contiguous()
+                        wav = self.eng.hift.forward(mel, it["render"][4], it["render"][5])
+                        it["rfut"].set_result((toks, mel, wav))
+                    mark = torch.cuda.Event()
+                    mark.record(self.stream)
+                    ahead.append(mark)
+                    if len(ahead) > self.AHEAD:
+                        ahead.popleft().synchronize()
+        except BaseException as e:
+            with self._cv:
+                self._dead = e
+                held = [w for w in self._waiting] + [j[0] for j in jobs.values()] + ([item] if item is not None else [])
+                self._waiting.clear()
+            for it in held:
+                if not it["rfut"].done():
+                    it["rfut"].set_exception(e)
+
+
 class PipelinedSynth:
 
     JOIN_QUANTUM = 16
     JOIN_AHEAD = 2
+    AUTOTUNE_RENDER_JOIN = os.environ.get("ASTTS_PIPE_RENDER_JOIN", "1") != "0"
 
     def __init__(self, engine, lm_depth: int = 2, lm_priority: int = -1, render_priority: int = 0, streams=None,
                  cobatch: int = 1, render_depth: int = 1, pipe_classes=None, front_prefill: Optional[bool] = None,
-                 stagger_ms: Optional[float] = None, wide_lm: bool = False, join: bool = False):
+                 stagger_ms: Optional[float] = None, wide_lm: bool = False, join: bool = False, render_join: bool = False):
         self.eng = engine
         self.depth = max(1, int(lm_depth))
         self.render_depth = rd = max(1, int(render_depth))
@@ -234,11 +365,15 @@
         lm_ = engine.lm
         self._chains = [_JoinChain(lm_, dev, self.s_lm[c], c, self.JOIN_QUANTUM, self.JOIN_AHEAD, lm_.body.center)
                         for c in range(self.depth)] if self.join else []
+        self.render_join = bool(render_join) and rd == 1
+        self._renderer = _JoinRender(engine, self.s_render) if self.render_join else None
 
     def close(self) -> None:
         for ch in self._chains:
             ch.close()
         self._chains = []
+        if self._renderer is not None:
+            self._renderer.close()
         self._pool.shutdown(wait=True)
 
     @classmethod
@@ -255,13 +390,15 @@
                 if join and (cfg_[1] != 1 or wide_lm):
                     continue
                 tried.append(tuple(cfg_) + ("join",) if join else cfg_)
+                if join and cls.AUTOTUNE_RENDER_JOIN and len(cfg_) < 3:
+                    tried.append(tuple(cfg_) + ("join", "render_join"))
         for cfg_ in tried:
-            join = cfg_[-1] == "join"
-            depth, cob, rdep = (tuple(cfg_[:-1] if join else cfg_) + (1,))[:3]
+            join, rjoin = "join" in cfg_, "render_join" in cfg_
+            depth, cob, rdep = (tuple(c for c in cfg_ if not isinstance(c, str)) + (1,))[:3]
             for _ in range(trials):
                 lm_prio = int(os.environ.get("ASTTS_PIPE_LM_PRIORITY", "0"))
                 pipe = cls(engine, lm_depth=depth, lm_priority=lm_prio, render_priority=0, cobatch=cob, render_depth=rdep,
-                           pipe_classes=classes if rdep == 1 and lm_prio == 0 else None, wide_lm=wide_lm, join=join)
+                           pipe_classes=classes if rdep == 1 and lm_prio == 0 else None, wide_lm=wide_lm, join=join, render_join=rjoin)
                 with torch.cuda.stream(pipe.front_stream):
                     for _ in range((depth + 1) * cob):
                         if front is not None:
@@ -278,7 +415,7 @@
                     torch.cuda.synchronize(engine.device)
                 dt = (time.perf_counter() - t0) / steps
                 if verbose:
-                    print(f"PipelinedSynth.autotune: depth {depth} cobatch {cob} render streams {rdep} join {join}: {dt * 1e3:.1f} ms/batch", flush=True)
+                    print(f"PipelinedSynth.autotune: depth {depth} cobatch {cob} render streams {rdep} join {join} render join {rjoin}: {dt * 1e3:.1f} ms/batch", flush=True)
                 if dt < best_dt:
                     best, best_dt = pipe, dt
                 if not per_cfg or per_cfg[-1][2] != cfg_:
@@ -334,8 +471,17 @@
         fut = self._pool.submit(lm_stage)
         for k, g in enumerate(group):
             g["fut"], g["k"] = fut, k
+            self._to_renderer(g)
+
+    def _to_renderer(self, item) -> None:
+        if self._renderer is not None:
+            self._renderer.submit(item, item["ready"])
 
     def _render(self, item):
+        if self._renderer is not None:
+            out = item["rfut"].result()
+            record_streams(out, torch.cuda.current_stream(self.eng.device))
+            return out
         parts, ev = item["fut"].result()
         toks = parts[item["k"]]
         cur = torch.cuda.current_stream(self.eng.device)
@@ -352,11 +498,19 @@
     def submit(self, text, text_lens, lm_spk, lm_prompt_tokens, n_tokens, uniforms, flow_prompt_tokens, flow_prompt_mel,
                flow_spk, z, phase0, noise):
         cur = torch.cuda.current_stream(self.eng.device)
-        for sr in self.s_renders:
-            sr.wait_stream(cur)
         item = {"lm": LmArgs(text, text_lens, lm_spk, lm_prompt_tokens, n_tokens, uniforms),
                 "render": (flow_prompt_tokens, flow_prompt_mel, flow_spk, z, phase0, noise), "fut": None, "k": 0}
+        if self._renderer is None:
+            for sr in self.s_renders:
+                sr.wait_stream(cur)
+        else:
+            item["ready"] = torch.cuda.Event()
+            item["ready"].record(cur)
         if self.join and self._join_submit(item):
+            if self._renderer is not None:
+                rfut = self._fifo[0].get("rfut")
+                done = rfut is not None and (rfut.done() or len(self._fifo) > 2 * self.depth + _JoinRender.SLOTS)
+                return self._render(self._fifo.popleft()) if done else None
             return self._render(self._fifo.popleft()) if len(self._fifo) > 2 * self.depth else None
         if self._pending and not self._compatible(self._pending[0]["lm"], item["lm"]):
             self._launch_group()
@@ -392,6 +546,7 @@
             raise RuntimeError("PipelinedSynth: no decode chain can take the batch although none holds one")
         self._fifo.append(item)
         item["fut"] = chain.submit(state, lm_args)
+        self._to_renderer(item)
         return True
 
     def _compatible(self, a: LmArgs, b: LmArgs) -> bool:
diff --git a/autostyle-tts_amd/csrc/flow_engine.hip b/autostyle-tts_amd/csrc/flow_engine.hip
--- a/autostyle-tts_amd/csrc/flow_engine.hip
+++ b/autostyle-tts_amd/csrc/flow_engine.hip
@@ -1,4 +1,6 @@
 #include "common.h"
+#include "flow_session.h"
+#include "../../include/session/astts_flow_session.h"
 
 #include <vector>
 
@@ -135,20 +137,58 @@
     return o;
 }
 
+struct Seg {
+    float* x;
+    const float *mu, *spk, *cond;
+    int seq0, b;
+    float dt, cfg_rate;
+};
+
 struct Ctx {
     const astts_flow* h;
     Buffers B;
     int b2, T;
     bool full;
     astts_stream_t st;
-
+    const Seg* seg;
+    int n_seg;
+
+    int gemm1(const void* x, int x16, const astts_weight_t& w, const float* residual, void* out, int out16, int64_t m,
+              int t_in, int t_out, int stride, int pad, int act) const {
+        return astts_op_gemm(x, x16, w.w, w.bias, residual, nullptr, out, out16, m, w.n, w.cin, w.cin_pad, w.taps, w.cin, w.n,
+                             residual ? w.n : 0, t_in, t_out, stride, 1, pad, act, 1.0f, 0.1f, nullptr, st);
+    }
     int gemm(const void* x, int x16, const astts_weight_t& w, const float* residual, void* out, int out16, int64_t m,
              int t_in, int t_out, int stride, int pad, int act) const {
-        return astts_op_gemm(x, x16, w.w, w.bias, residual, nullptr, out, out16, m, w.n, w.cin, w.cin_pad, w.taps, w.cin, w.n,
-                             residual ? w.n : 0, t_in, t_out, stride, 1, pad, act, 1.0f, 0.1f, nullptr, st);
+        if (n_seg == 1) return gemm1(x, x16, w, residual, out, out16, m, t_in, t_out, stride, pad, act);
+        for (int i = 0; i < n_seg; ++i) {
+            const int64_t s0 = seg[i].seq0, nb = 2 * (int64_t)seg[i].b;
+            RUN(gemm1((const char*)x + s0 * t_in * w.cin * (x16 ? 2 : 4), x16, w, residual ? residual + s0 * t_out * w.n : nullptr,
+                      (char*)out + s0 * t_out * w.n * (out16 ? 2 : 4), out16, nb * t_out, t_in, t_out, stride, pad, act));
+        }
+        return ASTTS_OK;
     }
     int linear(const void* x, int x16, const astts_weight_t& w, const float* residual, void* out, int out16, int64_t m, int act) const {
-        return gemm(x, x16, w, residual, out, out16, m, (int)m, (int)m, 1, 0, act);
+        return gemm1(x, x16, w, residual, out, out16, m, (int)m, (int)m, 1, 0, act);
+    }
+    int linear_seq(const void* x, int x16, const astts_weight_t& w, const float* residual, void* out, int out16, int t, int act) const {
+        if (n_seg == 1) return linear(x, x16, w, residual, out, out16, (int64_t)b2 * t, act);
+        for (int i = 0; i < n_seg; ++i) {
+            const int64_t r0 = (int64_t)seg[i].seq0 * t, m = 2 * (int64_t)seg[i].b * t;
+            RUN(linear((const char*)x + r0 * w.cin * (x16 ? 2 : 4), x16, w, residual ? residual + r0 * w.n : nullptr,
+                       (char*)out + r0 * w.n * (out16 ? 2 : 4), out16, m, act));
+        }
+        return ASTTS_OK;
+    }
+    int gnorm(const float* x, const int* lens, const float* gw, const float* gb, const float* add_bc, void* y, int y16, int t) const {
+        const int C = h->cfg.channels, G = h->cfg.groups;
+        for (int i = 0; i < n_seg; ++i) {
+            const int64_t s0 = n_seg == 1 ? 0 : seg[i].seq0;
+            const int nb = n_seg == 1 ? b2 : 2 * seg[i].b;
+            RUN(astts_op_groupnorm(x + s0 * t * C, lens + s0, gw, gb, add_bc ? add_bc + s0 * C : nullptr, (char*)y + s0 * t * C * (y16 ? 2 : 4),
+                                   y16, nb, t, C, G, 1e-5f, 1, B.gn_ws, B.gn_ws_bytes, st));
+        }
+        return ASTTS_OK;
     }
     int mask(float* x, const int* lens, int t, int c) const {
         if (full) return ASTTS_OK;
@@ -157,7 +197,7 @@
 
     int resnet(const astts_flow_resnet_t& r, const float* tproj, const float* x, const int* lens, int t, float* out,
                const void* next_w = nullptr, uint32_t next_bytes = 0) const {
-        const int C = h->cfg.channels, G = h->cfg.groups;
+        const int G = h->cfg.groups;
         const int64_t rows = (int64_t)b2 * t;
         if (r.c1_frag && r.c2_frag && r.res_frag && astts_op_resnet_conv_supported(r.c1.cin, r.c1.n, G, r.c1.taps) &&
             astts_op_resnet_conv_supported(r.c2.cin, r.c2.n, G, r.c2.taps) && astts_op_resnet_conv_supported(r.res.cin, r.res.n, G, r.res.taps)) {
@@ -170,9 +210,9 @@
                                         nullptr, lens, b2, t, r.res.cin, r.res.taps, 1e-5f, next_w, next_bytes, st);
         }
         RUN(gemm(x, 0, r.c1, nullptr, B.r1, 0, rows, t, t, 1, 1, ASTTS_ACT_NONE));
-        RUN(astts_op_groupnorm(B.r1, lens, r.g1_w, r.g1_b, tproj, B.r1h, 1, b2, t, C, G, 1e-5f, 1, B.gn_ws, B.gn_ws_bytes, st));
+        RUN(gnorm(B.r1, lens, r.g1_w, r.g1_b, tproj, B.r1h, 1, t));
         RUN(gemm(B.r1h, 1, r.c2, nullptr, B.r2, 0, rows, t, t, 1, 1, ASTTS_ACT_NONE));
-        RUN(astts_op_groupnorm(B.r2, lens, r.g2_w, r.g2_b, nullptr, B.r3, 0, b2, t, C, G, 1e-5f, 1, B.gn_ws, B.gn_ws_bytes, st));
+        RUN(gnorm(B.r2, lens, r.g2_w, r.g2_b, nullptr, B.r3, 0, t));
         return gemm(x, 0, r.res, B.r3, out, 0, rows, t, t, 1, 0, ASTTS_ACT_NONE);
     }
 
@@ -188,21 +228,32 @@
                                         (w.wo_frag && w.w1_frag && w.w2_frag) ? 3 : 0, st));
         } else {
             RUN(astts_op_layernorm(p, w.n1_w, w.n1_b, B.n16, 1, rows, C, C, C, 1e-5f, 0.0f, st));
-            RUN(linear(B.n16, 1, w.qkv, nullptr, B.qkv16, 1, rows, ASTTS_ACT_NONE));
+            RUN(linear_seq(B.n16, 1, w.qkv, nullptr, B.qkv16, 1, t, ASTTS_ACT_NONE));
             RUN(astts_op_attn_mha(B.qkv16, B.qkv16 + hd, B.qkv16 + 2 * hd, 1, lens, B.a16, 1, b2, heads, t, 3 * hd, 3 * hd, hd,
                                   0.125f, st));
         }
         const bool ffn = w.w1_frag && w.w2_frag && astts_op_tfm_ffn_fused_supported(C, w.w1.n);
-        if (ffn && w.wo_frag && (hd == 256 || hd == 512))
-            return astts_op_tfm_ffn_fused(p, w.w1_frag, w.w1.bias, w.w2_frag, w.w2.bias, p, rows, C, w.w1.n, 1e-5f, B.a16, w.wo_frag,
-                                          w.wo.bias, hd, next_w, next_bytes, st);
-        RUN(linear(B.a16, 1, w.wo, p, q, 0, rows, ASTTS_ACT_NONE));
-        if (ffn)
-            return astts_op_tfm_ffn_fused(q, w.w1_frag, w.w1.bias, w.w2_frag, w.w2.bias, p, rows, C, w.w1.n, 1e-5f, nullptr, nullptr, nullptr, 0, nullptr, 0,
-                                          st);
+        if (ffn && w.wo_frag && (hd == 256 || hd == 512)) {
+            for (int i = 0; i < n_seg; ++i) {
+                const int64_t r0 = n_seg == 1 ? 0 : (int64_t)seg[i].seq0 * t, m = n_seg == 1 ? rows : 2 * (int64_t)seg[i].b * t;
+                const bool last = i + 1 == n_seg;
+                RUN(astts_op_tfm_ffn_fused(p + r0 * C, w.w1_frag, w.w1.bias, w.w2_frag, w.w2.bias, p + r0 * C, m, C, w.w1.n, 1e-5f, B.a16 + r0 * hd,
+                                           w.wo_frag, w.wo.bias, hd, last ? next_w : nullptr, last ? next_bytes : 0u, st));
+            }
+            return ASTTS_OK;
+        }
+        RUN(linear_seq(B.a16, 1, w.wo, p, q, 0, t, ASTTS_ACT_NONE));
+        if (ffn) {
+            for (int i = 0; i < n_seg; ++i) {
+                const int64_t r0 = n_seg == 1 ? 0 : (int64_t)seg[i].seq0 * t, m = n_seg == 1 ? rows : 2 * (int64_t)seg[i].b * t;
+                RUN(astts_op_tfm_ffn_fused(q + r0 * C, w.w1_frag, w.w1.bias, w.w2_frag, w.w2.bias, p + r0 * C, m, C, w.w1.n, 1e-5f, nullptr, nullptr,
+                                           nullptr, 0, nullptr, 0, st));
+            }
+            return ASTTS_OK;
+        }
         RUN(astts_op_layernorm(q, w.n3_w, w.n3_b, B.n16, 1, rows, C, C, C, 1e-5f, 0.0f, st));
-        RUN(linear(B.n16, 1, w.w1, nullptr, B.f16, 1, rows, ASTTS_ACT_GELU));
-        return linear(B.f16, 1, w.w2, q, p, 0, rows, ASTTS_ACT_NONE);
+        RUN(linear_seq(B.n16, 1, w.w1, nullptr, B.f16, 1, t, ASTTS_ACT_GELU));
+        return linear_seq(B.f16, 1, w.w2, q, p, 0, t, ASTTS_ACT_NONE);
     }
 };
 
@@ -251,52 +302,50 @@
     return carve(h, b, t, nullptr, nullptr);
 }
 
-int astts_flow_solve(astts_flow_t* h, float* x, const float* mu, const float* spk, const float* cond, const int32_t* lens,
-                     int32_t b, int32_t t, int32_t n_steps, const float* t_host, const float* dt_host, float cfg_rate,
-                     void* workspace, size_t workspace_bytes, astts_stream_t stream) {
-    ASTTS_REQUIRE(h && x && mu && spk && cond && t_host && dt_host && workspace, ASTTS_ERR_INVALID, "astts_flow_solve: null argument");
-    ASTTS_REQUIRE(b >= 1 && t >= 2 && n_steps >= 1, ASTTS_ERR_INVALID, "astts_flow_solve: b=%d t=%d n_steps=%d", b, t, n_steps);
-    ASTTS_REQUIRE(workspace_bytes >= astts_flow_workspace_bytes(h, b, t) && ((uintptr_t)workspace & 255) == 0,
-                  ASTTS_ERR_WORKSPACE, "astts_flow_solve: workspace too small or misaligned");
+}
+
+namespace {
+
+struct TimeBufs {
+    float *tv, *temb0, *temb1, *temb2, *tproj;
+};
+
+int time_path(const Ctx& k, const TimeBufs& T, const float* t_host, int steps, int b2) {
+    const astts_flow* h = k.h;
     const astts_flow_config_t& c = h->cfg;
-    hipStream_t st = (hipStream_t)stream;
-    Ctx k;
-    k.h = h;
-    k.b2 = 2 * b;
-    k.T = t;
-    k.full = lens == nullptr;
-    k.st = stream;
-    carve(h, b, t, (char*)workspace, &k.B);
+    hipStream_t st = (hipStream_t)k.st;
+    const int64_t trows = (int64_t)steps * b2;
+    for (int j = 0; j < steps; ++j) {
+        hipLaunchKernelGGL(flow_fill_time, dim3((b2 + 63) / 64), dim3(64), 0, st, T.tv + (size_t)j * b2, t_host[j], b2);
+        ASTTS_CHECK_LAUNCH();
+    }
+    RUN(astts_op_time_embedding(T.tv, T.temb0, (int)trows, c.time_in, 1000.0f, k.st));
+    RUN(k.linear(T.temb0, 0, c.t1, nullptr, T.temb1, 0, trows, ASTTS_ACT_SILU));
+    RUN(k.linear(T.temb1, 0, c.t2, nullptr, T.temb2, 0, trows, ASTTS_ACT_NONE));
+    RUN(astts_op_elementwise(ASTTS_EL_MISH, T.temb2, nullptr, nullptr, nullptr, T.temb2, trows * c.time_dim, 1, c.time_dim, 0.0f, 0.0f, k.st));
+    size_t rj = 0;
+    for (const std::vector<astts_flow::Block>* grp : {&h->down, &h->mid, &h->up})
+        for (const astts_flow::Block& blk : *grp)
+            RUN(k.linear(T.temb2, 0, blk.res.mlp, nullptr, T.tproj + (rj++) * (size_t)trows * c.channels, 0, trows, ASTTS_ACT_NONE));
+    return ASTTS_OK;
+}
+
+int estimator_pass(const Ctx& k, const float* tproj, size_t tproj_stride, const int* lens_full, const int* lens_half) {
+    const astts_flow* h = k.h;
+    const astts_flow_config_t& c = h->cfg;
+    hipStream_t st = (hipStream_t)k.st;
     const Buffers& B = k.B;
-    const int b2 = k.b2, C = c.channels, mel = c.mel;
+    const int b2 = k.b2, t = k.T, C = c.channels, mel = c.mel;
     const int t_half = (t - 1) / 2 + 1;
-
-    hipLaunchKernelGGL(flow_fill_lens, dim3((b2 + 63) / 64), dim3(64), 0, st, lens, B.lens_full, B.lens_half, b, t);
-    ASTTS_CHECK_LAUNCH();
-
-    for (int s = 0; s < n_steps; ++s) {
-      const int s0 = s - s % FLOW_MAX_STEPS, sl = s - s0;
-      const int64_t trows = (int64_t)(n_steps - s0 < FLOW_MAX_STEPS ? n_steps - s0 : FLOW_MAX_STEPS) * b2;
-      if (sl == 0) {
-        for (int j = 0; j < (int)(trows / b2); ++j) {
-            hipLaunchKernelGGL(flow_fill_time, dim3((b2 + 63) / 64), dim3(64), 0, st, B.tv + (size_t)j * b2, t_host[s0 + j], b2);
-            ASTTS_CHECK_LAUNCH();
-        }
-        RUN(astts_op_time_embedding(B.tv, B.temb0, (int)trows, c.time_in, 1000.0f, st));
-        RUN(k.linear(B.temb0, 0, c.t1, nullptr, B.temb1, 0, trows, ASTTS_ACT_SILU));
-        RUN(k.linear(B.temb1, 0, c.t2, nullptr, B.temb2, 0, trows, ASTTS_ACT_NONE));
-        RUN(astts_op_elementwise(ASTTS_EL_MISH, B.temb2, nullptr, nullptr, nullptr, B.temb2, trows * c.time_dim, 1, c.time_dim, 0.0f, 0.0f, st));
-        size_t rj = 0;
-        for (const std::vector<astts_flow::Block>* grp : {&h->down, &h->mid, &h->up})
-            for (const astts_flow::Block& blk : *grp)
-                RUN(k.linear(B.temb2, 0, blk.res.mlp, nullptr, B.tproj + (rj++) * (size_t)trows * C, 0, trows, ASTTS_ACT_NONE));
-      }
       {
         size_t ri = 0;
-        auto tproj_of = [&]() { return B.tproj + ((ri++) * (size_t)trows + (size_t)sl * b2) * C; };
-        hipLaunchKernelGGL(flow_pack_input, dim3(grid_for((int64_t)b2 * t * 4 * mel)), dim3(256), 0, st, x, mu, spk, cond,
-                           B.lens_full, B.xin, b, t, mel);
-        ASTTS_CHECK_LAUNCH();
+        auto tproj_of = [&]() { return tproj + (ri++) * tproj_stride; };
+        for (int i = 0; i < k.n_seg; ++i) {
+            const Seg& g = k.seg[i];
+            hipLaunchKernelGGL(flow_pack_input, dim3(grid_for((int64_t)2 * g.b * t * 4 * mel)), dim3(256), 0, st, g.x, g.mu, g.spk, g.cond,
+                               lens_full + g.seq0, B.xin + (size_t)g.seq0 * t * 4 * mel, g.b, t, mel);
+            ASTTS_CHECK_LAUNCH();
+        }
 
         float* pool[6];
         for (int i = 0; i < 6; ++i) pool[i] = B.pool[i];
@@ -310,7 +359,7 @@
         int n_skips = 0;
         const float* block_in = B.xin;
         int tt = t;
-        const int* L = B.lens_full;
+        const int* L = lens_full;
 
         const uint32_t qkv_bytes = 3u * (uint32_t)c.heads * 64u * (uint32_t)C * 2u;
         for (size_t i = 0; i < h->down.size(); ++i) {
@@ -332,7 +381,7 @@
             if (blk.kind == ASTTS_FLOW_RESAMPLE_DOWN) {
                 RUN(k.gemm(cur, 0, blk.resample, nullptr, nxt, 0, (int64_t)b2 * t_half, tt, t_half, 2, 1, ASTTS_ACT_NONE));
                 tt = t_half;
-                L = B.lens_half;
+                L = lens_half;
             } else {
                 RUN(k.gemm(cur, 0, blk.resample, nullptr, nxt, 0, (int64_t)b2 * tt, tt, tt, 1, 1, ASTTS_ACT_NONE));
             }
@@ -387,16 +436,265 @@
             }
         }
         float* fin = const_cast<float*>(up_src);
-        RUN(k.mask(fin, B.lens_full, t, C));
+        RUN(k.mask(fin, lens_full, t, C));
         RUN(k.gemm(fin, 0, c.fin_c, nullptr, B.r1, 0, (int64_t)b2 * t, t, t, 1, 1, ASTTS_ACT_NONE));
-        RUN(astts_op_groupnorm(B.r1, B.lens_full, c.fin_g_w, c.fin_g_b, nullptr, B.r3, 0, b2, t, C, c.groups, 1e-5f, 1, B.gn_ws,
-                               B.gn_ws_bytes, st));
+        RUN(k.gnorm(B.r1, lens_full, c.fin_g_w, c.fin_g_b, nullptr, B.r3, 0, t));
         RUN(k.gemm(B.r3, 0, c.fin_p, nullptr, B.d, 0, (int64_t)b2 * t, t, t, 1, 0, ASTTS_ACT_NONE));
-        RUN(k.mask(B.d, B.lens_full, t, mel));
-        RUN(astts_op_elementwise(ASTTS_EL_CFG_EULER, x, B.d, nullptr, nullptr, x, (int64_t)b * t * mel, t, mel, dt_host[s], cfg_rate, st));
+        RUN(k.mask(B.d, lens_full, t, mel));
+        for (int i = 0; i < k.n_seg; ++i) {
+            const Seg& g = k.seg[i];
+            RUN(astts_op_elementwise(ASTTS_EL_CFG_EULER, g.x, B.d + (size_t)g.seq0 * t * mel, nullptr, nullptr, g.x, (int64_t)g.b * t * mel, t, mel,
+                                     g.dt, g.cfg_rate, k.st));
+        }
       }
-    }
-    return ASTTS_OK;
-}
-
-}
+    return ASTTS_OK;
+}
+
+}
+
+struct FlowJoinTable {
+    const float* tproj[astts::FlowSessionPlan::kSlots];
+    const int* lens_full[astts::FlowSessionPlan::kSlots];
+    const int* lens_half[astts::FlowSessionPlan::kSlots];
+    int seq0[astts::FlowSessionPlan::kSlots], b2[astts::FlowSessionPlan::kSlots], trows[astts::FlowSessionPlan::kSlots],
+        step[astts::FlowSessionPlan::kSlots];
+    int n;
+};
+
+__global__ __launch_bounds__(256) void flow_join_assemble(FlowJoinTable T, float* __restrict__ tproj_out, int* __restrict__ lens_full,
+                                                         int* __restrict__ lens_half, int nseq, int n_res, int C) {
+    const int64_t total = (int64_t)n_res * nseq * C;
+    for (int64_t i = (int64_t)blockIdx.x * blockDim.x + threadIdx.x; i < total; i += (int64_t)gridDim.x * blockDim.x) {
+        const int cc = (int)(i % C);
+        const int seq = (int)((i / C) % nseq);
+        const int ri = (int)(i / ((int64_t)C * nseq));
+        int k = 0;
+        while (k + 1 < T.n && seq >= T.seq0[k] + T.b2[k]) ++k;
+        const int j = seq - T.seq0[k];
+        tproj_out[i] = T.tproj[k][((int64_t)ri * T.trows[k] + (int64_t)T.step[k] * T.b2[k] + j) * C + cc];
+        if (i < nseq) {
+            int kk = 0;
+            while (kk + 1 < T.n && (int)i >= T.seq0[kk] + T.b2[kk]) ++kk;
+            lens_full[i] = T.lens_full[kk][(int)i - T.seq0[kk]];
+            lens_half[i] = T.lens_half[kk][(int)i - T.seq0[kk]];
+        }
+    }
+}
+
+struct astts_flow_session {
+    astts_flow* h;
+    astts::FlowSessionPlan plan;
+    astts_stream_t st;
+    Buffers B;
+    struct Slot {
+        Seg seg;
+        TimeBufs T;
+        int *lens_full, *lens_half;
+        bool full;
+        float dt[FLOW_MAX_STEPS];
+    } slot[astts::FlowSessionPlan::kSlots];
+    int passes, carried;
+};
+
+namespace {
+
+size_t carve_session(const astts_flow* h, int t, int n_slots, int rows_max, int steps_max, char* base, astts_flow_session* S) {
+    const astts_flow_config_t& c = h->cfg;
+    size_t o = carve(h, rows_max, t, base, S ? &S->B : nullptr);
+    auto take = [&](size_t bytes) {
+        void* p = base ? base + o : nullptr;
+        o = align_up(o + bytes, 256);
+        return p;
+    };
+    const size_t n_res = h->down.size() + h->mid.size() + h->up.size();
+    const size_t trows = (size_t)steps_max * 2 * rows_max;
+    for (int i = 0; i < n_slots; ++i) {
+        astts_flow_session::Slot tmp;
+        astts_flow_session::Slot& X = S ? S->slot[i] : tmp;
+        X.T.tv = (float*)take(sizeof(float) * trows);
+        X.T.temb0 = (float*)take(sizeof(float) * trows * c.time_in);
+        X.T.temb1 = (float*)take(sizeof(float) * trows * c.time_dim);
+        X.T.temb2 = (float*)take(sizeof(float) * trows * c.time_dim);
+        X.T.tproj = (float*)take(sizeof(float) * n_res * trows * c.channels);
+        X.lens_full = (int*)take(sizeof(int) * 2 * rows_max);
+        X.lens_half = (int*)take(sizeof(int) * 2 * rows_max);
+    }
+    return o;
+}
+
+}
+
+extern "C" {
+
+int astts_flow_solve(astts_flow_t* h, float* x, const float* mu, const float* spk, const float* cond, const int32_t* lens,
+                     int32_t b, int32_t t, int32_t n_steps, const float* t_host, const float* dt_host, float cfg_rate,
+                     void* workspace, size_t workspace_bytes, astts_stream_t stream) {
+    ASTTS_REQUIRE(h && x && mu && spk && cond && t_host && dt_host && workspace, ASTTS_ERR_INVALID, "astts_flow_solve: null argument");
+    ASTTS_REQUIRE(b >= 1 && t >= 2 && n_steps >= 1, ASTTS_ERR_INVALID, "astts_flow_solve: b=%d t=%d n_steps=%d", b, t, n_steps);
+    ASTTS_REQUIRE(workspace_bytes >= astts_flow_workspace_bytes(h, b, t) && ((uintptr_t)workspace & 255) == 0,
+                  ASTTS_ERR_WORKSPACE, "astts_flow_solve: workspace too small or misaligned");
+    hipStream_t st = (hipStream_t)stream;
+    Seg seg{x, mu, spk, cond, 0, b, 0.0f, cfg_rate};
+    Ctx k;
+    k.h = h;
+    k.b2 = 2 * b;
+    k.T = t;
+    k.full = lens == nullptr;
+    k.st = stream;
+    k.seg = &seg;
+    k.n_seg = 1;
+    carve(h, b, t, (char*)workspace, &k.B);
+    const Buffers& B = k.B;
+    const int b2 = k.b2, C = h->cfg.channels;
+
+    hipLaunchKernelGGL(flow_fill_lens, dim3((b2 + 63) / 64), dim3(64), 0, st, lens, B.lens_full, B.lens_half, b, t);
+    ASTTS_CHECK_LAUNCH();
+
+    const TimeBufs T{B.tv, B.temb0, B.temb1, B.temb2, B.tproj};
+    for (int s = 0; s < n_steps; ++s) {
+        const int s0 = s - s % FLOW_MAX_STEPS, sl = s - s0;
+        const int steps = n_steps - s0 < FLOW_MAX_STEPS ? n_steps - s0 : FLOW_MAX_STEPS;
+        if (sl == 0) RUN(time_path(k, T, t_host + s0, steps, b2));
+        seg.dt = dt_host[s];
+        RUN(estimator_pass(k, B.tproj + (size_t)sl * b2 * C, (size_t)steps * b2 * C, B.lens_full, B.lens_half));
+    }
+    return ASTTS_OK;
+}
+
+size_t astts_flow_session_bytes(const astts_flow_t* h, int32_t t, int32_t n_slots, int32_t rows_max, int32_t steps_max) {
+    astts::FlowSessionPlan p;
+    if (!h || p.init(t, n_slots, rows_max, steps_max) != astts::FLOW_SESSION_OK || steps_max > FLOW_MAX_STEPS) return 0;
+    return carve_session(h, t, n_slots, rows_max, steps_max, nullptr, nullptr);
+}
+
+int astts_flow_session_create(astts_flow_t* h, int32_t t, int32_t n_slots, int32_t rows_max, int32_t steps_max, void* workspace,
+                              size_t workspace_bytes, astts_stream_t stream, astts_flow_session_t** out) {
+    ASTTS_REQUIRE(h && workspace && out, ASTTS_ERR_INVALID, "astts_flow_session_create: null argument");
+    astts::FlowSessionPlan p;
+    ASTTS_REQUIRE(p.init(t, n_slots, rows_max, steps_max) == astts::FLOW_SESSION_OK && steps_max <= FLOW_MAX_STEPS, ASTTS_ERR_INVALID,
+                  "astts_flow_session_create: t=%d n_slots=%d rows_max=%d steps_max=%d", t, n_slots, rows_max, steps_max);
+    ASTTS_REQUIRE(workspace_bytes >= astts_flow_session_bytes(h, t, n_slots, rows_max, steps_max) && ((uintptr_t)workspace & 255) == 0,
+                  ASTTS_ERR_WORKSPACE, "astts_flow_session_create: workspace too small or misaligned");
+    astts_flow_session* s = new astts_flow_session();
+    s->h = h;
+    s->plan = p;
+    s->st = stream;
+    s->passes = s->carried = 0;
+    carve_session(h, t, n_slots, rows_max, steps_max, (char*)workspace, s);
+    *out = s;
+    return ASTTS_OK;
+}
+
+int astts_flow_session_destroy(astts_flow_session_t* s) {
+    delete s;
+    return ASTTS_OK;
+}
+
+int astts_flow_session_can_admit(const astts_flow_session_t* s, int32_t b, int32_t t, int32_t n_steps) {
+    return s ? s->plan.admissible(b, t, n_steps) : astts::FLOW_SESSION_ERR_ARG;
+}
+
+int astts_flow_session_admit(astts_flow_session_t* s, float* x, const float* mu, const float* spk, const float* cond, const int32_t* lens,
+                             int32_t b, int32_t t, int32_t n_steps, const float* t_host, const float* dt_host, float cfg_rate,
+                             int32_t* slot_out) {
+    ASTTS_REQUIRE(s && x && mu && spk && cond && t_host && dt_host && slot_out, ASTTS_ERR_INVALID, "astts_flow_session_admit: null argument");
+    const int slot = s->plan.admissible(b, t, n_steps);
+    ASTTS_REQUIRE(slot >= 0, ASTTS_ERR_INVALID, "astts_flow_session_admit: b=%d t=%d n_steps=%d is not admissible now (%d)", b, t, n_steps, slot);
+    astts_flow_session::Slot& X = s->slot[slot];
+    X.seg = Seg{x, mu, spk, cond, 0, b, 0.0f, cfg_rate};
+    X.full = lens == nullptr;
+    for (int i = 0; i < n_steps; ++i) X.dt[i] = dt_host[i];
+    hipLaunchKernelGGL(flow_fill_lens, dim3((2 * b + 63) / 64), dim3(64), 0, (hipStream_t)s->st, lens, X.lens_full, X.lens_half, b, t);
+    ASTTS_CHECK_LAUNCH();
+    Ctx k;
+    k.h = s->h;
+    k.B = s->B;
+    k.b2 = 2 * b;
+    k.T = t;
+    k.full = X.full;
+    k.st = s->st;
+    k.seg = &X.seg;
+    k.n_seg = 1;
+    RUN(time_path(k, X.T, t_host, n_steps, 2 * b));
+    s->plan.admit(b, t, n_steps);
+    *slot_out = slot;
+    return ASTTS_OK;
+}
+
+int astts_flow_session_step(astts_flow_session_t* s, int32_t n_passes, uint32_t* finished_mask_out) {
+    ASTTS_REQUIRE(s && finished_mask_out && n_passes >= 1, ASTTS_ERR_INVALID, "astts_flow_session_step: bad argument");
+    using astts::FlowSessionPlan;
+    const int C = s->h->cfg.channels;
+    const int n_res = (int)(s->h->down.size() + s->h->mid.size() + s->h->up.size());
+    uint32_t done = 0;
+    *finished_mask_out = 0;
+    for (int p = 0; p < n_passes && s->plan.n_active() > 0; ++p) {
+        const int nseq = s->plan.layout();
+        Seg segs[FlowSessionPlan::kSlots];
+        int of[FlowSessionPlan::kSlots];
+        int n = 0;
+        bool full = true;
+        for (int i = 0; i < s->plan.n_slots; ++i) {
+            const astts::FlowSlot& ps = s->plan.s[i];
+            if (!ps.active) continue;
+            segs[n] = s->slot[i].seg;
+            segs[n].seq0 = ps.seq0;
+            segs[n].dt = s->slot[i].dt[ps.step];
+            full = full && s->slot[i].full;
+            of[n++] = i;
+        }
+        Ctx k;
+        k.h = s->h;
+        k.B = s->B;
+        k.b2 = nseq;
+        k.T = s->plan.t;
+        k.full = full;
+        k.st = s->st;
+        k.seg = segs;
+        k.n_seg = n;
+        if (n == 1) {
+            const astts_flow_session::Slot& X = s->slot[of[0]];
+            const astts::FlowSlot& ps = s->plan.s[of[0]];
+            RUN(estimator_pass(k, X.T.tproj + (size_t)ps.step * nseq * C, (size_t)ps.n_steps * nseq * C, X.lens_full, X.lens_half));
+        } else {
+            FlowJoinTable T{};
+            T.n = n;
+            for (int j = 0; j < n; ++j) {
+                const astts::FlowSlot& ps = s->plan.s[of[j]];
+                T.tproj[j] = s->slot[of[j]].T.tproj;
+                T.lens_full[j] = s->slot[of[j]].lens_full;
+                T.lens_half[j] = s->slot[of[j]].lens_half;
+                T.seq0[j] = ps.seq0;
+                T.b2[j] = 2 * ps.b;
+                T.trows[j] = ps.n_steps * 2 * ps.b;
+                T.step[j] = ps.step;
+            }
+            hipLaunchKernelGGL(flow_join_assemble, dim3(grid_for((int64_t)n_res * nseq * C)), dim3(256), 0, (hipStream_t)s->st, T, s->B.tproj,
+                               s->B.lens_full, s->B.lens_half, nseq, n_res, C);
+            ASTTS_CHECK_LAUNCH();
+            RUN(estimator_pass(k, s->B.tproj, (size_t)nseq * C, s->B.lens_full, s->B.lens_half));
+        }
+        s->passes += 1;
+        s->carried += n;
+        done |= s->plan.advance();
+    }
+    *finished_mask_out = done;
+    return ASTTS_OK;
+}
+
+int astts_flow_session_state(const astts_flow_session_t* s, int32_t* out8) {
+    ASTTS_REQUIRE(s && out8, ASTTS_ERR_INVALID, "astts_flow_session_state: null argument");
+    int mask = 0;
+    for (int i = 0; i < astts::FlowSessionPlan::kSlots; ++i) {
+        const astts::FlowSlot& ps = s->plan.s[i];
+        mask |= ps.active << i;
+        out8[4 + i] = ps.active ? ps.n_steps - ps.step : 0;
+    }
+    out8[0] = mask;
+    out8[1] = s->plan.rows_active();
+    out8[2] = s->passes;
+    out8[3] = s->carried;
+    return ASTTS_OK;
+}
+
+}
diff --git a/autostyle-tts_amd/csrc/flow_session.h b/autostyle-tts_amd/csrc/flow_session.h
--- /dev/null
+++ b/autostyle-tts_amd/csrc/flow_session.h
@@ -0,0 +1,82 @@
+#pragma once
+#include <cstdint>
+
+namespace astts {
+
+struct FlowSlot {
+    int active;
+    int b;
+    int n_steps, step;
+    int seq0;
+};
+
+enum { FLOW_SESSION_OK = 0, FLOW_SESSION_ERR_ARG = -1, FLOW_SESSION_ERR_T = -2, FLOW_SESSION_ERR_FULL = -3, FLOW_SESSION_ERR_ROWS = -4,
+       FLOW_SESSION_ERR_STEPS = -5 };
+
+struct FlowSessionPlan {
+    static constexpr int kSlots = 4;
+    int t = 0, n_slots = 0, rows_max = 0, steps_max = 0;
+    FlowSlot s[kSlots] = {};
+
+    int init(int t_, int n_slots_, int rows_max_, int steps_max_) {
+        if (t_ < 2 || n_slots_ < 1 || n_slots_ > kSlots || rows_max_ < 1 || steps_max_ < 1) return FLOW_SESSION_ERR_ARG;
+        t = t_;
+        n_slots = n_slots_;
+        rows_max = rows_max_;
+        steps_max = steps_max_;
+        for (FlowSlot& x : s) x = FlowSlot{};
+        return FLOW_SESSION_OK;
+    }
+
+    int n_active() const {
+        int n = 0;
+        for (int i = 0; i < n_slots; ++i) n += s[i].active;
+        return n;
+    }
+    int rows_active() const {
+        int n = 0;
+        for (int i = 0; i < n_slots; ++i) n += s[i].active ? s[i].b : 0;
+        return n;
+    }
+
+    int admissible(int b, int bt, int n_steps) const {
+        if (b < 1 || bt < 2 || n_steps < 1) return FLOW_SESSION_ERR_ARG;
+        if (bt != t) return FLOW_SESSION_ERR_T;
+        if (n_steps > steps_max) return FLOW_SESSION_ERR_STEPS;
+        if (b > rows_max - rows_active()) return FLOW_SESSION_ERR_ROWS;
+        for (int i = 0; i < n_slots; ++i)
+            if (!s[i].active) return i;
+        return FLOW_SESSION_ERR_FULL;
+    }
+
+    int admit(int b, int bt, int n_steps) {
+        const int slot = admissible(b, bt, n_steps);
+        if (slot < 0) return slot;
+        s[slot] = FlowSlot{1, b, n_steps, 0, 0};
+        return slot;
+    }
+
+    int layout() {
+        int seq = 0;
+        for (int i = 0; i < n_slots; ++i) {
+            if (!s[i].active) continue;
+            s[i].seq0 = seq;
+            seq += 2 * s[i].b;
+        }
+        return seq;
+    }
+
+    unsigned advance() {
+        unsigned done = 0;
+        for (int i = 0; i < n_slots; ++i) {
+            if (!s[i].active) continue;
+            if (++s[i].step >= s[i].n_steps) {
+                s[i].active = 0;
+                done |= 1u << i;
+            }
+        }
+        return done;
+    }
+};
+
+}
diff --git a/include/session/astts_flow_session.h b/include/session/astts_flow_session.h
--- /dev/null
+++ b/include/session/astts_flow_session.h
@@ -0,0 +1,25 @@
+#ifndef ASTTS_FLOW_SESSION_H
+#define ASTTS_FLOW_SESSION_H
+#include "../astts.h"
+
+#ifdef __cplusplus
+extern "C" {
+#endif
+
+typedef struct astts_flow_session astts_flow_session_t;
+
+size_t astts_flow_session_bytes(const astts_flow_t* h, int32_t t, int32_t n_slots, int32_t rows_max, int32_t steps_max);
+int astts_flow_session_create(astts_flow_t* h, int32_t t, int32_t n_slots, int32_t rows_max, int32_t steps_max, void* workspace,
+                              size_t workspace_bytes, astts_stream_t stream, astts_flow_session_t** out);
+int astts_flow_session_destroy(astts_flow_session_t* s);
+int astts_flow_session_can_admit(const astts_flow_session_t* s, int32_t b, int32_t t, int32_t n_steps);
+int astts_flow_session_admit(astts_flow_session_t* s, float* x, const float* mu, const float* spk, const float* cond, const int32_t* lens,
+                             int32_t b, int32_t t, int32_t n_steps, const float* t_host, const float* dt_host, float cfg_rate,
+                             int32_t* slot_out);
+int astts_flow_session_step(astts_flow_session_t* s, int32_t k, uint32_t* finished_mask_out);
+int astts_flow_session_state(const astts_flow_session_t* s, int32_t* out8);
+
+#ifdef __cplusplus
+}
+#endif
+#endif
```
